# rafaelgmv/Distributed-Autonomous-Exploration-and-Mapping

Hardware: AMD Instinct MI355X
Metric: beam-cell updates/sec + frontier-extract ms on 16384² grid (higher is better)
Workload: dtype int32/u32 ray math + fp32 log-odds (fp64 endpoints)

## Files before the change

### distributed-autonomous-exploration-and-mapping_amd/csrc/dm_api.cpp

```cpp
#include <math.h>
#include <stdarg.h>
#include <stdio.h>
#include <string.h>

#include <algorithm>
#include <new>
#include <string>
#include <vector>

#include "dm_internal.h"

#include <stdlib.h>

hipError_t dm_sync_all(dm_grid* g) {
  for (hipStream_t s : {g->stream, g->fe_stream, g->pass_stream, g->big_stream}) {
    if (!s) continue;
    const hipError_t e = hipStreamSynchronize(s);
    if (e != hipSuccess) return e;
  }
  g->p_pending = false;
  for (auto& f : g->fw) f.busy_pending = false;
  return hipSuccess;
}

hipError_t dm_copy_shards(dm_grid* g) {
  const size_t bytes = sizeof(unsigned long long) * kShards * kShardWords;
  hipError_t e = hipMemcpyAsync(g->h_sh, g->iw[g->iw_cur].sh, bytes, hipMemcpyDeviceToHost, g->stream);
  if (e == hipSuccess)
    e = hipMemcpyAsync(g->h_sh + kShards * kShardWords, g->fsh, bytes, hipMemcpyDeviceToHost, g->stream);
  return e;
}

namespace {
thread_local std::string t_err;

bool dm_env_on(const char* name) {
  const char* v = getenv(name);
  return v && v[0] == '1';
}


struct HostCluster {
  long long label, size, sum_x, sum_y;
};

template <class T>
int dev_alloc(T** p, int64_t count, const char* what) {
  if (*p) { (void)hipFree(*p); *p = nullptr; }
  if (count <= 0) count = 1;
  hipError_t e = hipMalloc((void**)p, sizeof(T) * (size_t)count);
  if (e != hipSuccess) {
    *p = nullptr;
    return dm_set_error(e == hipErrorOutOfMemory ? DM_ERR_OOM : DM_ERR_HIP,
                        "hipMalloc(%s, %lld bytes): %s", what,
                        (long long)(sizeof(T) * (size_t)count), hipGetErrorString(e));
  }
  return DM_OK;
}

template <class T>
void dev_free(T*& p) {
  if (p) (void)hipFree(p);
  p = nullptr;
}

template <class T>
int dev_grow(T** p, int64_t* cap, int64_t n, const char* what) {
  if (n <= *cap) return DM_OK;
  *cap = 0;
  const int rc = dev_alloc(p, n, what);
  if (!rc) *cap = n;
  return rc;
}

int64_t ceil_div(int64_t a, int64_t b) { return (a + b - 1) / b; }

int validate_params(const dm_params* p) {
  if (!p) return dm_set_error(DM_ERR_INVALID_ARG, "params is NULL");
  if (p->width <= 0 || p->height <= 0 || p->width > (1ll << 30) || p->height > (1ll << 30))
    return dm_set_error(DM_ERR_INVALID_ARG, "width/height must be in [1, 2^30] (got %lld x %lld)",
                        (long long)p->width, (long long)p->height);
  if (!(p->resolution > 0.0) || !isfinite(p->resolution))
    return dm_set_error(DM_ERR_INVALID_ARG, "resolution must be finite and > 0");
  if (!isfinite(p->origin_x) || !isfinite(p->origin_y))
    return dm_set_error(DM_ERR_INVALID_ARG, "origin must be finite");
  if (!(p->range_min >= 0.0f) || !(p->range_max > 0.0f) || !isfinite(p->range_max))
    return dm_set_error(DM_ERR_INVALID_ARG, "need 0 <= range_min and finite range_max > 0");
  if ((double)p->range_max / p->resolution > 16384.0)
    return dm_set_error(DM_ERR_INVALID_ARG,
                        "range_max / resolution must be <= 16384 cells (rays longer than that "
                        "are outside the kernels' integer bounds)");
  if (!isfinite(p->l_occ) || !isfinite(p->l_free) || !isfinite(p->l_min) || !isfinite(p->l_max) ||
      !(p->l_min <= p->l_max))
    return dm_set_error(DM_ERR_INVALID_ARG, "log-odds constants must be finite with l_min <= l_max");
  if (isnan(p->occ_thresh) || isnan(p->free_thresh))
    return dm_set_error(DM_ERR_INVALID_ARG, "occ_thresh / free_thresh must not be NaN");
  if (p->band_row0 < 0 || p->band_row0 >= p->height || p->band_row0 % DM_TILE != 0)
    return dm_set_error(DM_ERR_INVALID_ARG, "band_row0 must be in [0, height) and a multiple of %d",
                        DM_TILE);
  int64_t R = p->band_rows > 0 ? p->band_rows : p->height - p->band_row0;
  if (R <= 0 || p->band_row0 + R > p->height)
    return dm_set_error(DM_ERR_INVALID_ARG, "band_rows out of range");
  if (ceil_div(p->width, DM_TILE) * ceil_div(R, DM_TILE) > (1ll << 30))
    return dm_set_error(DM_ERR_INVALID_ARG, "too many tiles");
  if (p->min_frontier_size < 0) return dm_set_error(DM_ERR_INVALID_ARG, "min_frontier_size < 0");
  return DM_OK;
}

int grow_integrate(dm_grid* g, int32_t S, int32_t N) {
  const int64_t nb = (int64_t)S * N;
  const int64_t chunks = dm_integrate_chunks(g, nb);
  const int64_t per_beam = 2 * (g->nmax / DM_TILE) + 8 + 4 * chunks;
  const int64_t blocks = ceil_div(nb * chunks, 256);
  if (nb > g->beams_cap || blocks > g->blk_cap) {
    const int64_t nbc = std::max<int64_t>(nb, g->beams_cap);
    const int64_t bc = std::max<int64_t>(blocks, g->blk_cap);
    int rc = 0;
    for (auto& w : g->iw) {
      if (!rc) rc = dev_alloc(&w.beams, nbc, "beams");
      if (!rc) rc = dev_alloc(&w.blk_hist, bc * 1024, "per-block tile histograms");
      if (!rc) rc = dev_alloc(&w.blk_n, bc, "per-block histogram sizes");
    }
    if (rc) { g->beams_cap = g->blk_cap = 0; return rc; }
    g->beams_cap = nbc;
    g->blk_cap = bc;
  }
  const int64_t segs = nb * per_beam;
  if (segs > g->segs_cap) {
    for (auto& w : g->iw) {
      int rc = dev_alloc(&w.pieces, segs, "ray pieces");
      if (rc) { g->segs_cap = 0; return rc; }
    }
    g->segs_cap = segs;
  }
  const int64_t side = ceil_div(2 * (int64_t)g->nmax + 1, DM_TILE) + 1;
  int64_t act = std::min<int64_t>(g->NT, std::min<int64_t>(segs, (int64_t)S * side * side));
  if (act < 1) act = 1;
  if (act > g->act_cap) {
    int rc = 0;
    for (auto& w : g->iw) {
      if (!rc) rc = dev_alloc(&w.act_raw, act * kShards, "first-touch lists");
      if (!rc) rc = dev_alloc(&w.litems, act, "light work items");
    }
    if (rc) { g->act_cap = 0; return rc; }
    g->act_cap = act;
  }
  const int64_t chunk = kIntegrateChunk;
  const int64_t heavy = std::max<int64_t>(1, std::min<int64_t>(g->act_cap, segs / (kIntegrateMedium + 1) + 1));
  const int64_t hitems = segs / chunk + segs / (chunk + 1) + 2;
  if (hitems > g->hitem_cap) {
    for (auto& w : g->iw) {
      int rc = dev_alloc(&w.hitems, hitems, "heavy work items");
      if (rc) { g->hitem_cap = 0; return rc; }
    }
    g->hitem_cap = hitems;
  }
  if (heavy > g->heavy_cap) {
    for (auto& w : g->iw) {
      int rc = dev_alloc(&w.heavy_list, heavy, "heavy tiles");
      if (!rc) rc = dev_alloc(&w.slabs, heavy * 2 * DM_TILE * DM_TILE, "heavy-tile slabs");
      if (!rc) rc = dev_alloc(&w.heavy_done, heavy, "heavy-tile item tickets");
      if (rc) { g->heavy_cap = 0; return rc; }
      DM_HIP(hipMemset(w.slabs, 0, sizeof(uint32_t) * (size_t)(heavy * 2 * DM_TILE * DM_TILE)));
      DM_HIP(hipMemset(w.heavy_done, 0, sizeof(int32_t) * (size_t)heavy));
    }
    g->heavy_cap = heavy;
  }
  if (2 * (int64_t)N > g->trig_cap) {
    int rc = dev_alloc(&g->trig, 2 * (int64_t)N, "trig table");
    if (rc) return rc;
    g->trig_cap = 2 * (int64_t)N;
    g->trig_n = -1;
  }
  return DM_OK;
}

int ensure_trig(dm_grid* g, int32_t N, float amin, float inc) {
  if (N == g->trig_n && amin == g->trig_amin && inc == g->trig_inc) return DM_OK;
  DM_HIP(dm_sync_all(g));
  std::vector<double> t(2 * (size_t)std::max(N, 1));
  for (int32_t i = 0; i < N; ++i) {
    const double phi = (double)amin + (double)i * (double)inc;
    t[2 * i] = cos(phi);
    t[2 * i + 1] = sin(phi);
  }
  if (N > 0) DM_HIP(hipMemcpy(g->trig, t.data(), sizeof(double) * 2 * N, hipMemcpyHostToDevice));
  g->trig_n = N;
  g->trig_amin = amin;
  g->trig_inc = inc;
  return DM_OK;
}

}

int dm_grow_bucket_sort(dm_grid* g, int64_t n) {
  if (n <= g->bs_cap) return DM_OK;
  int rc = dev_alloc(&g->bs_key, n, "row-sort keys");
  if (!rc) rc = dev_alloc(&g->bs_key2, n, "row-sort keys");
  if (!rc) rc = dev_alloc(&g->bs_idx, n, "row-sort indices");
  if (!rc) rc = dev_alloc(&g->bs_idx2, n, "row-sort indices");
  if (!rc && g->rs_rows < g->H) {
    rc = dev_alloc(&g->rs_cnt, g->H, "row-sort counters");
    if (!rc) rc = dev_alloc(&g->rs_off, g->H + 1, "row-sort offsets");
    if (!rc) rc = dev_alloc(&g->rs_status, g->H / 8192 + 2, "row-sort workgroup totals");
    if (!rc) {
      DM_HIP(hipMemset(g->rs_cnt, 0, sizeof(int32_t) * (size_t)g->H));
      g->rs_rows = g->H;
    }
  }
  if (rc) { g->bs_cap = 0; return rc; }
  g->bs_cap = n;
  return DM_OK;
}

namespace {

int grow_slots(dm_grid* g, int64_t need) {
  int64_t cap = std::max<int64_t>(need, 2 * g->slot_cap);
  if (cap < (1 << 16)) cap = 1 << 16;
  cap = ceil_div(cap, kShards) * kShards;
  int rc = dev_alloc(&g->slot_label, cap, "slot labels");
  for (auto& f : g->fw)
    if (!rc) rc = dev_alloc(&f.slot_parent, cap, "slot parents");
  g->slot_parent = g->fw[g->fparity].slot_parent;
  if (!rc) rc = dev_alloc(&g->slot_root, cap, "slot roots");
  if (!rc) rc = dev_alloc(&g->slot_own, 3 * cap, "slot sums");
  if (!rc) rc = dev_alloc(&g->slot_acc, 3 * cap, "slot totals");
  if (!rc) rc = dev_alloc(&g->clusters, 4 * cap, "clusters");
  for (int sl = 0; sl <= dm_grid::kRbSlots && !rc; ++sl) {
    dm_cluster* base = g->rb[sl].out_clu ? g->rb[sl].out_clu - kRbRecords : nullptr;
    rc = dev_alloc(&base, cap + kRbRecords, "sorted clusters");
    g->rb[sl].out_clu = base ? base + kRbRecords : nullptr;
  }
  ++g->rb_gen;
  g->out_clu = g->rb[g->rb_head].out_clu;
  if (!rc) rc = dev_alloc(&g->slot_k, cap, "slot cluster index");
  if (!rc) rc = dev_alloc(&g->rank_of, cap, "cluster sorted position");
  if (!rc) rc = dm_grow_bucket_sort(g, cap);
  if (rc) return rc;
  g->slot_cap = cap;
  return DM_OK;
}

int grow_host_out(dm_grid* g, int slot, int64_t need) {
  dm_grid::RbSlot& r = g->rb[slot];
  if (need <= r.h_out_cap) return DM_OK;
  int64_t cap = std::max<int64_t>(need, 2 * r.h_out_cap);
  if (r.h_out) (void)hipHostFree(r.h_out - kRbHostRecords);
  r.h_out = nullptr;
  r.h_out_cap = 0;
  dm_raw_record* base = nullptr;
  DM_HIP(hipHostMalloc((void**)&base, sizeof(dm_raw_record) * (size_t)(cap + kRbHostRecords),
                       hipHostMallocMapped | hipHostMallocCoherent));
  dm_raw_record* dbase = nullptr;
  const hipError_t e = hipHostGetDevicePointer((void**)&dbase, base, 0);
  if (e != hipSuccess) {
    (void)hipHostFree(base);
    return dm_hip_check(e, "hipHostGetDevicePointer(cluster readback)");
  }
  r.h_out = base + kRbHostRecords;
  r.h_out_dev = dbase + kRbHostRecords;
  r.h_out_cap = cap;
  return DM_OK;
}

int copy_clusters(dm_grid* g, bool sorted, int64_t n, int64_t nw, int64_t have,
                  const dm_cluster* d_sorted, const long long* d_raw, dm_cluster* out) {
  if (sorted) {
    have = std::min<int64_t>(have, nw);
    const double ox = g->p.origin_x, oy = g->p.origin_y, res = g->p.resolution;
    for (int64_t i = 0; i < have; ++i) {
      const dm_raw_record& q = g->h_out[i];
      dm_cluster& c = out[i];
      c.label = q.label;
      c.size = q.size;
      c.sum_x = q.sum_x;
      c.sum_y = q.sum_y;
      c.cx_m = dm_centroid(ox, q.sum_x, q.size, res);
      c.cy_m = dm_centroid(oy, q.sum_y, q.size, res);
    }
    if (nw > have)
      DM_HIP(hipMemcpy(out + have, d_sorted + have, sizeof(dm_cluster) * (size_t)(nw - have),
                       hipMemcpyDeviceToHost));
    return DM_OK;
  }
  std::vector<HostCluster> hc((size_t)n);
  if (n > 0) DM_HIP(hipMemcpy(hc.data(), d_raw, sizeof(HostCluster) * (size_t)n, hipMemcpyDeviceToHost));
  std::sort(hc.begin(), hc.end(), [](const HostCluster& a, const HostCluster& b) { return a.label < b.label; });
  for (int64_t i = 0; i < nw; ++i) {
    dm_cluster& c = out[i];
    c.label = hc[i].label;
    c.size = hc[i].size;
    c.sum_x = hc[i].sum_x;
    c.sum_y = hc[i].sum_y;
    c.cx_m = dm_centroid(g->p.origin_x, c.sum_x, c.size, g->p.resolution);
    c.cy_m = dm_centroid(g->p.origin_y, c.sum_y, c.size, g->p.resolution);
  }
  return DM_OK;
}

void note_goal_source(dm_grid* g, int slot, int kind, int64_t n) {
  g->goal_slot = n >= 0 ? slot : -1;
  g->goal_kind = kind;
  g->goal_n = n;
  g->goal_epoch = kind == 1 ? g->rb[slot].wepoch : g->rb[slot].mepoch;
  g->goal_gen = g->rb_gen;
}

int grow_merge(dm_grid* g, int64_t n) {
  if (n <= g->m_cap) return DM_OK;
  int rc = dev_alloc(&g->m_parent, n, "merge parents");
  if (!rc) rc = dev_alloc(&g->m_label, n, "merge labels");
  if (!rc) rc = dev_alloc(&g->m_acc, 3 * n, "merge sums");
  if (!rc) rc = dev_alloc(&g->m_clu, 4 * n, "merged clusters");
  for (int sl = 0; sl <= dm_grid::kRbSlots && !rc; ++sl)
    rc = dev_alloc(&g->rb[sl].m_out, n, "merged clusters (sorted)");
  ++g->rb_gen;
  if (!rc) rc = dm_grow_bucket_sort(g, n);
  if (rc) { g->m_cap = 0; return rc; }
  g->m_cap = n;
  return DM_OK;
}

int check_grid(const dm_grid* g) {
  if (!g) return dm_set_error(DM_ERR_INVALID_ARG, "grid handle is NULL");
  return DM_OK;
}

int not_on_sharded(const dm_grid* g, const char* what) {
  if (g && g->sh)
    return dm_set_error(DM_ERR_INVALID_ARG, "%s is not available on a sharded handle (dm_create_sharded runs "
                                            "the band exchange itself)", what);
  return DM_OK;
}

int use_device(const dm_grid* g) {
  DM_HIP(hipSetDevice(g->device));
  return DM_OK;
}

int check_integrate_args(int32_t S, int32_t N, const void* poses, const void* ranges) {
  if (S < 0 || N < 0) return dm_set_error(DM_ERR_SHAPE, "S and N must be >= 0");
  if ((int64_t)S * N > (1ll << 31) - 1) return dm_set_error(DM_ERR_SHAPE, "S*N must be < 2^31");
  if (N > 65535) return dm_set_error(DM_ERR_SHAPE, "N must be <= 65535");
  if ((int64_t)S * N > 0 && (!poses || !ranges))
    return dm_set_error(DM_ERR_INVALID_ARG, "poses/ranges is NULL");
  return DM_OK;
}

int read_counters(dm_grid* g) {
  DM_HIP(dm_join_pass_stream(g));
  DM_HIP(hipMemcpyAsync(g->h_cnt, g->cnt, sizeof(unsigned long long) * CNT_N,
                        hipMemcpyDeviceToHost, g->stream));
  DM_HIP(hipMemcpyAsync(g->h_cnt + CNT_N, g->iw[g->iw_cur].cnt, sizeof(unsigned long long) * CNT_N,
                        hipMemcpyDeviceToHost, g->stream));
  DM_HIP(hipMemcpyAsync(g->h_cnt + 2 * CNT_N, g->fe_flag + kHaltWord, sizeof(unsigned long long),
                        hipMemcpyDeviceToHost, g->stream));
  DM_HIP(dm_copy_shards(g));
  DM_HIP(hipStreamSynchronize(g->stream));
  if (g->h_cnt[2 * CNT_N])
    return dm_set_error(DM_ERR_PIPELINE, "the overlapped pipeline's front-end hand-off timed out: a map "
                        "update was skipped; dm_reset the handle");
  return DM_OK;
}

int finish_counts(dm_grid* g, uint64_t* U, uint64_t* T) {
  int rc = read_counters(g);
  if (rc) return rc;
  const unsigned long long* ic = g->h_cnt + CNT_N;
  if (ic[CNT_IOVERFLOW]) {
    (void)hipMemset(g->iw[g->iw_cur].tile_count, 0, sizeof(int32_t) * (size_t)g->NT);
    return dm_set_error(DM_ERR_CAPACITY, "integrate workspace overflow (flags %llu: 1 first-touch "
                        "list, 2 pieces, 4 work lists)",
                        (unsigned long long)ic[CNT_IOVERFLOW]);
  }
  if (U) *U = dm_shard_sum(g->h_sh, SH_U);
  if (T) *T = dm_shard_sum(g->h_sh, SH_T);
  return DM_OK;
}

}

int dm_set_error(int code, const char* fmt, ...) {
  char buf[512];
  va_list ap;
  va_start(ap, fmt);
  vsnprintf(buf, sizeof buf, fmt, ap);
  va_end(ap);
  t_err = buf;
  return code;
}

int dm_hip_check(hipError_t e, const char* what) {
  return dm_set_error(e == hipErrorOutOfMemory ? DM_ERR_OOM : DM_ERR_HIP, "%s: %s (%d)", what,
                      hipGetErrorString(e), (int)e);
}

void dm_timer_begin(dm_grid* g, const char* name, KernelTimer* t, hipStream_t s) {
  if (!g->profile) return;
  t->name = name;
  t->stream = s ? s : g->stream;
  (void)hipEventCreate(&t->start);
  (void)hipEventCreate(&t->stop);
  (void)hipEventRecord(t->start, t->stream);
}

void dm_timer_end(dm_grid* g, KernelTimer* t) {
  if (!g->profile) return;
  (void)hipEventRecord(t->stop, t->stream);
  g->pending.push_back(*t);
  if (g->pending.size() > 4096) {
    int32_t n = 0;
    (void)dm_profile_read(g, nullptr, 0, &n);
  }
}

extern "C" {

const char* dm_last_error(void) { return t_err.c_str(); }
const char* dm_version(void) { return "dm 0.1.0 (gfx950, HIP)"; }
int dm_max_passes_in_flight(void) { return dm_grid::kRbSlots; }

int dm_default_params(dm_params* p, int64_t width, int64_t height) {
  if (!p) return dm_set_error(DM_ERR_INVALID_ARG, "params is NULL");
  memset(p, 0, sizeof *p);
  p->width = width;
  p->height = height;
  p->resolution = 0.05;
  p->origin_x = -0.5 * (double)width * p->resolution;
  p->origin_y = -0.5 * (double)height * p->resolution;
  p->range_min = 0.02f;
  p->range_max = 12.0f;
  p->l_occ = 0.85f;
  p->l_free = -0.4f;
  p->l_min = -2.0f;
  p->l_max = 3.5f;
  p->occ_thresh = 0.0f;
  p->free_thresh = 0.0f;
  p->min_frontier_size = 1;
  p->band_row0 = 0;
  p->band_rows = 0;
  return DM_OK;
}

int dm_create(dm_grid** out, const dm_params* p, int device) {
  if (!out) return dm_set_error(DM_ERR_INVALID_ARG, "out is NULL");
  *out = nullptr;
  int rc = validate_params(p);
  if (rc) return rc;
  int ndev = 0;
  hipError_t e = hipGetDeviceCount(&ndev);
  if (e != hipSuccess || ndev <= 0)
    return dm_set_error(DM_ERR_HIP, "no HIP device available (%s)", hipGetErrorString(e));
  if (device < 0 || device >= ndev)
    return dm_set_error(DM_ERR_INVALID_ARG, "device %d out of range [0, %d)", device, ndev);
  DM_HIP(hipSetDevice(device));
  dm_grid* g = new (std::nothrow) dm_grid();
  if (!g) return dm_set_error(DM_ERR_OOM, "host allocation failed");
  g->p = *p;
  if (g->p.band_rows <= 0) g->p.band_rows = p->height - p->band_row0;
  g->device = device;
  g->W = p->width;
  g->H = p->height;
  g->row0 = p->band_row0;
  g->R = g->p.band_rows;
  g->TX = ceil_div(g->W, DM_TILE);
  g->TY = ceil_div(g->R, DM_TILE);
  g->NT = g->TX * g->TY;
  g->nmax = (int32_t)ceil((double)p->range_max / p->resolution) + 2;
  const int64_t cells = g->W * g->R;
  auto fail = [&](int code) {
    dm_destroy(g);
    return code;
  };
  if ((rc = dev_alloc(&g->L, cells, "log-odds"))) return fail(rc);
  if ((rc = dev_alloc(&g->state, cells, "state"))) return fail(rc);
  for (auto& w : g->iw) {
    if ((rc = dev_alloc(&w.tile_count, g->NT, "tile counts"))) return fail(rc);
    if ((rc = dev_alloc(&w.tile_cur, g->NT, "tile bin cursors"))) return fail(rc);
    if ((rc = dev_alloc(&w.cnt, CNT_N, "integrate counters"))) return fail(rc);
    if ((rc = dev_alloc(&w.sh, kShards * kShardWords, "integrate shard counters"))) return fail(rc);
    DM_HIP(hipMemset(w.cnt, 0, sizeof(unsigned long long) * CNT_N));
    DM_HIP(hipMemset(w.sh, 0, sizeof(unsigned long long) * kShards * kShardWords));
  }
  if ((rc = dev_alloc(&g->tile_free, g->NT, "tile free counts"))) return fail(rc);
  if ((rc = dev_alloc(&g->fmask, g->NT * DM_TILE * 16, "tile free / unknown bit rows"))) return fail(rc);
  if ((rc = dev_alloc(&g->fedge, g->NT * 4, "tile unknown edge words"))) return fail(rc);
  if ((rc = dev_alloc(&g->tile_seen, g->NT, "tile seen flags"))) return fail(rc);
  if (const char* sp = getenv("DM_SPARSE_PIECES")) g->sparse_pieces = std::max(0, atoi(sp));
  const char* fm = getenv("DM_FMASK");
  g->fmask_mode = fm && !strcmp(fm, "on") ? 1 : (fm && !strcmp(fm, "off") ? 2 : 0);
  const char* fk = getenv("DM_FRONTIER_KERNEL");
  g->frontier_kernel = fk && !strcmp(fk, "wave") ? 1 : (fk && !strcmp(fk, "wg") ? 2 : 0);
  if (const char* sm = getenv("DM_SORT_MIN")) g->sort_min = std::max<int64_t>(0, atoll(sm));
  g->fault_gate = dm_env_on("DM_FAULT_GATE");
  if (const char* pr = getenv("DM_PLAN_MAX_ROUNDS")) g->plan_max_rounds = std::max<int64_t>(0, atoll(pr));
  for (auto& f : g->fw) {
    e = hipEventCreateWithFlags(&f.ev_split, hipEventDisableTiming | hipEventDisableSystemFence);
    if (e != hipSuccess) return fail(dm_hip_check(e, "hipEventCreate"));
    if ((rc = dev_alloc(&f.cnt, CNT_N, "frontier counters"))) return fail(rc);
    DM_HIP(hipMemset(f.cnt, 0, sizeof(unsigned long long) * CNT_N));
    if ((rc = dev_alloc(&f.fsh, kShards * kShardWords, "frontier shard counters"))) return fail(rc);
    DM_HIP(hipMemset(f.fsh, 0, sizeof(unsigned long long) * kShards * kShardWords));
    if ((rc = dev_alloc(&f.big_tiles, g->NT, "frontier big tiles"))) return fail(rc);
    if ((rc = dev_alloc(&f.fbits, g->NT * DM_TILE, "frontier bit rows"))) return fail(rc);
    if ((rc = dev_alloc(&f.edge_slot, 2 * g->W, "edge slots"))) return fail(rc);
  }
  if ((rc = dev_alloc(&g->fl_n, 48, "frontier list lengths"))) return fail(rc);
  for (int i = 0; i < 2; ++i) {
    if ((rc = dev_alloc(&g->flist[i], g->NT, "frontier tile list"))) return fail(rc);
    if ((rc = dev_alloc(&g->flist_n[i], 16, "frontier tile list length"))) return fail(rc);
    DM_HIP(hipMemset(g->flist_n[i], 0, sizeof(unsigned long long) * 16));
  }
  g->ftiles = g->flist[0];
  g->ftiles_n = g->flist_n[0];
  DM_HIP(hipMemset(g->fl_n, 0, sizeof(unsigned long long) * 48));
  if ((rc = dev_alloc(&g->bits_flag, 16, "bit-row hand-off word"))) return fail(rc);
  DM_HIP(hipMemset(g->bits_flag, 0, sizeof(unsigned long long) * 16));
  if ((rc = dev_alloc(&g->fe_flag, 16, "front-end completion words"))) return fail(rc);
  DM_HIP(hipMemset(g->fe_flag, 0, sizeof(unsigned long long) * 16));
  if ((rc = dev_alloc(&g->border, g->NT * 256, "frontier borders"))) return fail(rc);
  if ((rc = dev_alloc(&g->rel, 8 * g->NT, "tile-edge hand-off words"))) return fail(rc);
  DM_HIP(hipMemset(g->rel, 0, sizeof(unsigned long long) * 8 * (size_t)g->NT));
  if ((rc = dev_alloc(&g->edge_label, 2 * g->W, "edge labels"))) return fail(rc);
  if ((rc = dev_alloc(&g->halo, 2 * g->W, "halo rows"))) return fail(rc);
  if ((rc = grow_slots(g, std::max<int64_t>(1 << 16, kSlotsPerTile * g->NT)))) return fail(rc);
  dm_select_fw(g, g->fparity);
  for (int sl = 0; sl <= dm_grid::kRbSlots; ++sl)
    if ((rc = grow_host_out(g, sl, 1 << 14))) return fail(rc);
  dm_select_slot(g, 0);
  e = hipHostMalloc((void**)&g->h_cnt, sizeof(unsigned long long) * (2 * CNT_N + 1), hipHostMallocDefault);
  if (e != hipSuccess) return fail(dm_hip_check(e, "hipHostMalloc(counters)"));
  e = hipHostMalloc((void**)&g->h_sh, sizeof(unsigned long long) * 2 * kShards * kShardWords,
                    hipHostMallocDefault);
  if (e != hipSuccess) return fail(dm_hip_check(e, "hipHostMalloc(shard counters)"));
  if ((rc = dev_alloc(&g->m_cnt, 4, "merge counters"))) return fail(rc);
  e = hipHostMalloc((void**)&g->h_mcnt, sizeof(unsigned long long) * 4, hipHostMallocDefault);
  if (e != hipSuccess) return fail(dm_hip_check(e, "hipHostMalloc(merge counters)"));
  e = hipHostMalloc((void**)&g->h_hint, sizeof(unsigned long long) * 16, hipHostMallocMapped | hipHostMallocCoherent);
  if (e != hipSuccess) return fail(dm_hip_check(e, "hipHostMalloc(work hint)"));
  memset(g->h_hint, 0, sizeof(unsigned long long) * 16);
  e = hipHostGetDevicePointer((void**)&g->d_hint, g->h_hint, 0);
  if (e != hipSuccess) return fail(dm_hip_check(e, "hipHostGetDevicePointer(work hint)"));
  e = hipDeviceGetAttribute(&g->n_cu, hipDeviceAttributeMultiprocessorCount, device);
  if (e != hipSuccess) return fail(dm_hip_check(e, "hipDeviceGetAttribute(multiprocessor count)"));
  int prio_lo = 0, prio_hi = 0;
  (void)hipDeviceGetStreamPriorityRange(&prio_lo, &prio_hi);
  e = hipStreamCreateWithPriority(&g->stream, hipStreamNonBlocking, prio_hi);
  if (e != hipSuccess) return fail(dm_hip_check(e, "hipStreamCreate"));
  g->own_stream = true;
  e = hipStreamCreateWithPriority(&g->fe_stream, hipStreamNonBlocking, prio_lo);
  if (e != hipSuccess) return fail(dm_hip_check(e, "hipStreamCreate(front-end)"));
  e = hipStreamCreateWithPriority(&g->pass_stream, hipStreamNonBlocking, prio_hi);
  if (e != hipSuccess) return fail(dm_hip_check(e, "hipStreamCreate(pass)"));
  e = hipStreamCreateWithPriority(&g->big_stream, hipStreamNonBlocking, prio_hi);
  if (e != hipSuccess) return fail(dm_hip_check(e, "hipStreamCreate(big)"));
  for (hipEvent_t* ev : {&g->ev_fe, &g->ev_bits[0], &g->ev_bits[1], &g->iw[0].ev_free, &g->iw[1].ev_free,
                         &g->ev_bigfork, &g->ev_big, &g->flist_ev[0], &g->flist_ev[1]}) {
    e = hipEventCreateWithFlags(ev, hipEventDisableTiming | hipEventDisableSystemFence);
    if (e != hipSuccess) return fail(dm_hip_check(e, "hipEventCreate"));
  }
  for (auto& r : g->rb) {
    e = hipEventCreateWithFlags(&r.ev, hipEventDisableTiming);
    if (e != hipSuccess) return fail(dm_hip_check(e, "hipEventCreate"));
  }
  for (hipEvent_t& ev : g->ev_pose) {
    e = hipEventCreateWithFlags(&ev, hipEventDisableTiming);
    if (e != hipSuccess) return fail(dm_hip_check(e, "hipEventCreate"));
  }

  if ((rc = dm_reset(g))) return fail(rc);
  *out = g;
  return DM_OK;
}

int dm_destroy(dm_grid* g) {
  if (g && g->sh) return dm_sh_destroy(g);
  if (!g) return DM_OK;
  (void)hipSetDevice(g->device);
  (void)dm_sync_all(g);
  for (auto& t : g->pending) { (void)hipEventDestroy(t.start); (void)hipEventDestroy(t.stop); }
  for (hipEvent_t ev : {g->ev_fe, g->ev_bits[0], g->ev_bits[1], g->iw[0].ev_free, g->iw[1].ev_free,
                        g->ev_bigfork, g->ev_big, g->flist_ev[0], g->flist_ev[1]})
    if (ev) (void)hipEventDestroy(ev);
  for (auto& r : g->rb) {
    if (r.ev) (void)hipEventDestroy(r.ev);
    if (r.out_clu) (void)hipFree(r.out_clu - kRbRecords);
    if (r.h_out) (void)hipHostFree(r.h_out - kRbHostRecords);
    dev_free(r.m_out);
  }
  if (g->fe_stream) (void)hipStreamDestroy(g->fe_stream);
  if (g->pass_stream) (void)hipStreamDestroy(g->pass_stream);
  if (g->big_stream) (void)hipStreamDestroy(g->big_stream);
  for (auto& f : g->fw) {
    if (f.ev_split) (void)hipEventDestroy(f.ev_split);
    dev_free(f.cnt); dev_free(f.fsh); dev_free(f.big_tiles); dev_free(f.fbits);
    dev_free(f.edge_slot); dev_free(f.slot_parent);
  }
  dev_free(g->fl_n); dev_free(g->bits_flag);
  for (int i = 0; i < 2; ++i) { dev_free(g->flist[i]); dev_free(g->flist_n[i]); }
  for (int b = 0; b < 2; ++b) { dev_free(g->goal_k[b]); dev_free(g->goal_i[b]); }
  dev_free(g->goal_io); dev_free(g->goal_idx);
  dev_free(g->plan_cost); dev_free(g->plan_trav); dev_free(g->plan_travs); dev_free(g->plan_list[0]);
  dev_free(g->plan_list[1]); dev_free(g->plan_stamp); dev_free(g->plan_len); dev_free(g->plan_stat);
  dev_free(g->plan_src); dev_free(g->plan_qxy); dev_free(g->plan_qcost); dev_free(g->plan_qcell);
  dev_free(g->plan_path);
  if (g->h_plan) (void)hipHostFree(g->h_plan);
  dev_free(g->match_V); dev_free(g->match_kern); dev_free(g->match_tiles); dev_free(g->match_pose4);
  dev_free(g->match_trig); dev_free(g->match_ranges); dev_free(g->match_q); dev_free(g->match_vol);
  dev_free(g->match_out);
  for (auto& w : g->iw) {
    dev_free(w.pieces); dev_free(w.hitems); dev_free(w.litems); dev_free(w.heavy_list); dev_free(w.slabs);
    dev_free(w.heavy_done); dev_free(w.tile_count); dev_free(w.tile_cur); dev_free(w.cnt); dev_free(w.sh);
    dev_free(w.ranges);
    dev_free(w.beams); dev_free(w.blk_hist); dev_free(w.blk_n); dev_free(w.act_raw);
  }
  dev_free(g->L); dev_free(g->state); dev_free(g->fmask); dev_free(g->fedge); dev_free(g->tile_seen);
  dev_free(g->tile_free);
  dev_free(g->trig);
  dev_free(g->bs_key); dev_free(g->bs_key2); dev_free(g->bs_idx); dev_free(g->bs_idx2);
  dev_free(g->rs_cnt); dev_free(g->rs_off); dev_free(g->rs_status);
  dev_free(g->border); dev_free(g->rel); dev_free(g->slot_label); dev_free(g->slot_root);
  dev_free(g->slot_own); dev_free(g->slot_acc); dev_free(g->clusters); dev_free(g->cell_slot);
  dev_free(g->edge_label); dev_free(g->mask); dev_free(g->labels);
  dev_free(g->halo); dev_free(g->fe_flag);
  dev_free(g->slot_k); dev_free(g->rank_of); dev_free(g->m_parent); dev_free(g->m_label);
  dev_free(g->m_acc); dev_free(g->m_clu); dev_free(g->m_cnt);
  if (g->h_mcnt) (void)hipHostFree(g->h_mcnt);
  if (g->h_hint) (void)hipHostFree(g->h_hint);
  if (g->h_cnt) (void)hipHostFree(g->h_cnt);
  if (g->h_sh) (void)hipHostFree(g->h_sh);
  for (int i = 0; i < dm_grid::kPoseRing; ++i) {
    if (g->h_pose4[i]) (void)hipHostFree(g->h_pose4[i]);
    if (g->ev_pose[i]) (void)hipEventDestroy(g->ev_pose[i]);
  }
  if (g->stream && g->own_stream) (void)hipStreamDestroy(g->stream);
  delete g;
  return DM_OK;
}

int dm_reset(dm_grid* g) {
  if (g && g->sh) return dm_sh_reset(g);
  int rc = check_grid(g);
  if (rc || (rc = use_device(g))) return rc;
  const int64_t cells = g->W * g->R;
  DM_HIP(hipMemsetAsync(g->L, 0, sizeof(float) * (size_t)cells, g->stream));
  DM_HIP(hipMemsetAsync(g->state, 0xFF, (size_t)cells, g->stream));
  DM_HIP(dm_sync_all(g));
  for (auto& w : g->iw) DM_HIP(hipMemsetAsync(w.tile_count, 0, sizeof(int32_t) * (size_t)g->NT, g->stream));
  DM_HIP(hipMemsetAsync(g->tile_free, 0, sizeof(int32_t) * (size_t)g->NT, g->stream));
  if ((rc = dm_launch_recount(g))) return rc;
  for (auto& f : g->fw) DM_HIP(hipMemsetAsync(f.cnt, 0, sizeof(unsigned long long) * CNT_N, g->stream));
  DM_HIP(hipMemsetAsync(g->fe_flag + kHaltWord, 0, sizeof(unsigned long long), g->stream));
  DM_HIP(hipStreamSynchronize(g->stream));
  ++g->reset_seq;
  return DM_OK;
}

int dm_get_params(const dm_grid* g, dm_params* out) {
  int rc = check_grid(g);
  if (rc) return rc;
  if (!out) return dm_set_error(DM_ERR_INVALID_ARG, "out is NULL");
  *out = g->p;
  return DM_OK;
}

}

namespace {

int enqueue_host_integrate(dm_grid* g, int32_t S, const double* poses, int32_t N, const float* ranges,
                           float angle_min, float angle_increment) {
  int rc = 0;
  if ((rc = check_integrate_args(S, N, poses, ranges))) return rc;
  if ((rc = grow_integrate(g, S, N))) return rc;
  if ((rc = ensure_trig(g, N, angle_min, angle_increment))) return rc;
  const int64_t nb = (int64_t)S * N;
  hipStream_t fs = g->overlap ? g->fe_stream : g->stream;
  dm_grid::IntWs& w = g->iw[dm_next_set(g)];
  if (g->overlap) {
    DM_HIP(dm_mark_ws_free(g));
    DM_HIP(hipStreamWaitEvent(fs, w.free_wait ? w.free_wait : w.ev_free, 0));
  }
  if (nb > w.ranges_cap || (int64_t)S * 4 > g->h_pose_cap) {
    DM_HIP(dm_sync_all(g));
  }
  if (nb > w.ranges_cap) {
    if ((rc = dev_alloc(&w.ranges, nb, "ranges"))) return rc;
    w.ranges_cap = nb;
  }
  if ((int64_t)S * 4 > g->h_pose_cap) {
    for (int i = 0; i < dm_grid::kPoseRing; ++i) {
      if (g->h_pose4[i]) (void)hipHostFree(g->h_pose4[i]);
      g->h_pose4[i] = nullptr;
    }
    g->h_pose_cap = 0;
    for (int i = 0; i < dm_grid::kPoseRing; ++i) {
      DM_HIP(hipHostMalloc((void**)&g->h_pose4[i], sizeof(double) * 4 * (size_t)std::max(S, 1),
                           hipHostMallocMapped | hipHostMallocCoherent));
      DM_HIP(hipHostGetDevicePointer((void**)&g->h_pose4_dev[i], g->h_pose4[i], 0));
    }
    g->h_pose_cap = (int64_t)std::max(S, 1) * 4;
  }
  const int slot = g->pose_head;
  g->pose_head = (g->pose_head + 1) % dm_grid::kPoseRing;
  DM_HIP(hipEventSynchronize(g->ev_pose[slot]));
  double* hp = g->h_pose4[slot];
  for (int32_t s = 0; s < S; ++s) {
    const double x = poses[3 * s], y = poses[3 * s + 1], yaw = poses[3 * s + 2];
    hp[4 * s + 0] = x;
    hp[4 * s + 1] = y;
    hp[4 * s + 2] = cos(yaw);
    hp[4 * s + 3] = sin(yaw);
  }
  if (nb > 0)
    DM_HIP(hipMemcpyAsync(w.ranges, ranges, sizeof(float) * (size_t)nb, hipMemcpyHostToDevice, fs));
  if ((rc = dm_launch_integrate(g, S, g->h_pose4_dev[slot], N, w.ranges, g->trig))) return rc;
  DM_HIP(hipEventRecord(g->ev_pose[slot], fs));
  g->last_S = S;
  g->last_N = N;
  g->frontier_valid = false;
  ++g->integrate_seq;
  return DM_OK;
}

}

extern "C" {

int dm_integrate(dm_grid* g, int32_t S, const double* poses, int32_t N, const float* ranges,
                 float angle_min, float angle_increment, uint64_t* out_updates,
                 uint64_t* out_touched) {
  if (g && g->sh) return dm_sh_integrate(g, S, poses, N, ranges, angle_min, angle_increment, out_updates, out_touched);
  int rc = check_grid(g);
  if (rc || (rc = use_device(g))) return rc;
  if ((rc = enqueue_host_integrate(g, S, poses, N, ranges, angle_min, angle_increment))) return rc;
  return finish_counts(g, out_updates, out_touched);
}

int dm_integrate_async(dm_grid* g, int32_t S, const double* poses, int32_t N, const float* ranges,
                       float angle_min, float angle_increment) {
  if (g && g->sh) return dm_sh_integrate_async(g, S, poses, N, ranges, angle_min, angle_increment);
  int rc = check_grid(g);
  if (rc || (rc = use_device(g))) return rc;
  return enqueue_host_integrate(g, S, poses, N, ranges, angle_min, angle_increment);
}

int dm_integrate_device(dm_grid* g, int32_t S, const double* d_pose4, int32_t N,
                        const float* d_ranges, float angle_min, float angle_increment) {
  if (g && g->sh) return dm_sh_integrate_device(g, S, d_pose4, N, d_ranges, angle_min, angle_increment);
  int rc = check_grid(g);
  if (rc || (rc = use_device(g))) return rc;
  if ((rc = check_integrate_args(S, N, d_pose4, d_ranges))) return rc;
  if ((rc = grow_integrate(g, S, N))) return rc;
  if ((rc = ensure_trig(g, N, angle_min, angle_increment))) return rc;
  if ((rc = dm_launch_integrate(g, S, d_pose4, N, d_ranges, g->trig))) return rc;
  g->last_S = S;
  g->last_N = N;
  g->frontier_valid = false;
  ++g->integrate_seq;
  return DM_OK;
}

int dm_last_counts(dm_grid* g, uint64_t* updates, uint64_t* touched) {
  if (g && g->sh) return dm_sh_last_counts(g, updates, touched);
  int rc = check_grid(g);
  if (rc || (rc = use_device(g))) return rc;
  return finish_counts(g, updates, touched);
}

int dm_last_stats(dm_grid* g, uint64_t* out, int32_t cap, int32_t* n_out) {
  if (g && g->sh) return dm_sh_last_stats(g, out, cap, n_out);
  int rc = check_grid(g);
  if (rc || (rc = use_device(g))) return rc;
  if (cap > 0 && !out) return dm_set_error(DM_ERR_INVALID_ARG, "out is NULL");
  if ((rc = read_counters(g))) return rc;
  const unsigned long long* fs = g->h_sh + kShards * kShardWords;
  const unsigned long long* ic = g->h_cnt + CNT_N;
  const uint64_t items = ic[CNT_ITEMS] + ic[CNT_LITEMS] + ic[CNT_SITEMS];
  const uint64_t pieces = ic[CNT_SEGS];
  const uint64_t v[kNStats] = {dm_shard_sum(g->h_sh, SH_U),  dm_shard_sum(g->h_sh, SH_T),
                               dm_shard_sum(g->h_sh, SH_TH), pieces,
                               ic[CNT_ACTIVE],               items,
                               ic[CNT_HEAVY],                g->h_cnt[CNT_FL0],
                               dm_shard_sum(fs, SH_SLOT),    g->h_cnt[CNT_CLUSTERS],
                               ic[CNT_SITEMS]};
  for (int32_t i = 0; i < cap && i < kNStats; ++i) out[i] = v[i];
  if (n_out) *n_out = kNStats;
  return DM_OK;
}

int dm_get_state(dm_grid* g, int8_t* out) {
  if (g && g->sh) return (out ? dm_sh_get_state(g, out) : dm_set_error(DM_ERR_INVALID_ARG, "out is NULL"));
  int rc = check_grid(g);
  if (rc || (rc = use_device(g))) return rc;
  if (!out) return dm_set_error(DM_ERR_INVALID_ARG, "out is NULL");
  DM_HIP(hipMemcpyAsync(out, g->state, (size_t)(g->W * g->R), hipMemcpyDeviceToHost, g->stream));
  DM_HIP(hipStreamSynchronize(g->stream));
  return DM_OK;
}

int dm_get_logodds(dm_grid* g, float* out) {
  if (g && g->sh) return (out ? dm_sh_get_logodds(g, out) : dm_set_error(DM_ERR_INVALID_ARG, "out is NULL"));
  int rc = check_grid(g);
  if (rc || (rc = use_device(g))) return rc;
  if (!out) return dm_set_error(DM_ERR_INVALID_ARG, "out is NULL");
  DM_HIP(hipMemcpyAsync(out, g->L, sizeof(float) * (size_t)(g->W * g->R), hipMemcpyDeviceToHost,
                        g->stream));
  DM_HIP(hipStreamSynchronize(g->stream));
  return DM_OK;
}

int dm_set_logodds(dm_grid* g, const float* in) {
  if (g && g->sh) return (in ? dm_sh_set_logodds(g, in) : dm_set_error(DM_ERR_INVALID_ARG, "in is NULL"));
  int rc = check_grid(g);
  if (rc || (rc = use_device(g))) return rc;
  if (!in) return dm_set_error(DM_ERR_INVALID_ARG, "in is NULL");
  DM_HIP(hipStreamSynchronize(g->stream));
  DM_HIP(hipMemcpy(g->L, in, sizeof(float) * (size_t)(g->W * g->R), hipMemcpyHostToDevice));
  if ((rc = dm_launch_state_from_logodds(g))) return rc;
  DM_HIP(hipStreamSynchronize(g->stream));
  g->frontier_valid = false;
  ++g->integrate_seq;
  return DM_OK;
}

int dm_set_state(dm_grid* g, const int8_t* in) {
  if (g && g->sh) return (in ? dm_sh_set_state(g, in) : dm_set_error(DM_ERR_INVALID_ARG, "in is NULL"));
  int rc = check_grid(g);
  if (rc || (rc = use_device(g))) return rc;
  if (!in) return dm_set_error(DM_ERR_INVALID_ARG, "in is NULL");
  const int64_t cells = g->W * g->R;
  int8_t* d = nullptr;
  if ((rc = dev_alloc(&d, cells, "state staging"))) return rc;
  DM_HIP(hipStreamSynchronize(g->stream));
  hipError_t e = hipMemcpy(d, in, (size_t)cells, hipMemcpyHostToDevice);
  if (e == hipSuccess) {
    rc = dm_launch_set_state(g, d);
    if (!rc) e = hipStreamSynchronize(g->stream);
  }
  (void)hipFree(d);
  if (e != hipSuccess) return dm_hip_check(e, "dm_set_state");
  g->frontier_valid = false;
  ++g->integrate_seq;
  return rc;
}

int dm_frontiers(dm_grid* g, uint8_t* mask, int64_t* labels, dm_cluster* out, int64_t cap,
                 int64_t* n_out) {
  if (g && g->sh) return dm_sh_frontiers(g, mask, labels, out, cap, n_out);
  int rc = check_grid(g);
  if (rc || (rc = use_device(g))) return rc;
  if (cap < 0 || (cap > 0 && !out)) return dm_set_error(DM_ERR_INVALID_ARG, "bad cluster buffer");
  const int64_t cells = g->W * g->R;
  if (mask && !g->mask && (rc = dev_alloc(&g->mask, cells, "dense mask"))) return rc;
  if (labels && !g->cell_slot) {
    if ((rc = dev_alloc(&g->cell_slot, cells, "dense cell slots"))) return rc;
    if ((rc = dev_alloc(&g->labels, cells, "dense labels"))) return rc;
  }
  const int slot = dm_grid::kRbSync;
  dm_select_slot(g, slot);
  int64_t n = 0, copied = 0;
  for (int attempt = 0; attempt < 8; ++attempt) {
    rc = dm_launch_frontiers(g, mask != nullptr, labels != nullptr, &n, &copied);
    if (rc != DM_ERR_CAPACITY) break;
    if ((rc = grow_slots(g, n + n / 2 + 1024))) return rc;
    rc = DM_ERR_CAPACITY;
  }
  if (rc) return rc == DM_ERR_CAPACITY ? dm_set_error(rc, "frontier slot arrays kept overflowing") : rc;
  g->frontier_valid = true;
  const int64_t nw = std::min<int64_t>(n, cap);
  note_goal_source(g, slot, 1, g->h_cnt[CNT_SORTED] != 0 ? n : -1);
  if ((rc = copy_clusters(g, g->h_cnt[CNT_SORTED] != 0, n, nw, copied, g->out_clu, g->clusters, out)))
    return rc;
  if ((rc = grow_host_out(g, slot, n + n / 4 + 64))) return rc;
  if (mask) DM_HIP(hipMemcpy(mask, g->mask, (size_t)cells, hipMemcpyDeviceToHost));
  if (labels) DM_HIP(hipMemcpy(labels, g->labels, sizeof(int64_t) * (size_t)cells, hipMemcpyDeviceToHost));
  if (n_out) *n_out = n;
  if (n > cap) return dm_set_error(DM_ERR_CAPACITY, "%lld clusters, capacity %lld", (long long)n,
                                   (long long)cap);
  return DM_OK;
}

int dm_export_bytes(const dm_grid* g, int64_t rec_cap, int64_t* bytes) {
  if (int rc0 = not_on_sharded(g, "dm_export_bytes")) return rc0;
  int rc = check_grid(g);
  if (rc) return rc;
  if (!bytes || rec_cap < 0) return dm_set_error(DM_ERR_INVALID_ARG, "bytes is NULL or rec_cap < 0");
  *bytes = dm_export_nbytes(g->W, rec_cap);
  return DM_OK;
}

int dm_frontiers_export_device(dm_grid* g, void* d_export, int64_t rec_cap) {
  if (int rc0 = not_on_sharded(g, "dm_frontiers_export_device")) return rc0;
  int rc = check_grid(g);
  if (rc || (rc = use_device(g))) return rc;
  if (!d_export || rec_cap < 0) return dm_set_error(DM_ERR_INVALID_ARG, "d_export is NULL or rec_cap < 0");
  if (g->p.min_frontier_size > 1)
    return dm_set_error(DM_ERR_INVALID_ARG,
                        "export needs a band handle with min_frontier_size <= 1 (the size filter "
                        "applies to merged clusters)");
  dm_select_slot(g, g->rb_count < dm_grid::kRbSlots ? (g->rb_head + g->rb_count) % dm_grid::kRbSlots
                                                    : dm_grid::kRbSync);
  hipStream_t es = g->stream;
  if ((rc = dm_enqueue_frontiers(g, false, false, g->overlap, &es))) return rc;
  if ((rc = dm_launch_export(g, es, d_export, rec_cap))) return rc;
  if (es != g->stream) {
    dm_grid::FrWs& f = g->fw[g->fparity];
    DM_HIP(hipEventRecord(f.ev_split, es));
    f.busy = f.ev_split;
    f.busy_pending = true;
    f.busy_pass = g->fr_pass;
    g->p_tail = f.ev_split;
    g->p_pending = true;
    g->p_tail_pass = g->fr_pass;
  } else {
    DM_HIP(dm_mark_ws_free(g));
  }
  g->frontier_valid = true;
  return DM_OK;
}

int dm_exchange_stream(dm_grid* g, void** stream) {
  if (int rc0 = not_on_sharded(g, "dm_exchange_stream")) return rc0;
  int rc = check_grid(g);
  if (rc) return rc;
  if (!stream) return dm_set_error(DM_ERR_INVALID_ARG, "stream is NULL");
  *stream = (void*)dm_exchange_stream_of(g);
  return DM_OK;
}

namespace {

int claim_slot(dm_grid* g, int* slot) {
  if (g->rb_count == dm_grid::kRbSlots)
    return dm_set_error(DM_ERR_INVALID_ARG, "%d passes in flight: end the oldest first", dm_grid::kRbSlots);
  *slot = (g->rb_head + g->rb_count) % dm_grid::kRbSlots;
  dm_select_slot(g, *slot);
  return DM_OK;
}

int wait_oldest(dm_grid* g, int kind, const char* what) {
  if (!g->rb_count || g->rb[g->rb_head].kind != kind)
    return dm_set_error(DM_ERR_INVALID_ARG, "the oldest pass in flight is not a %s pass", what);
  DM_HIP(dm_event_wait(g->rb[g->rb_head].ev));
  if (kind == 1) {
    const uint64_t pass = g->rb[g->rb_head].pass;
    for (auto& f : g->fw)
      if (f.busy_pending && f.busy_pass <= pass) f.busy_pending = false;
    if (g->p_pending && g->p_tail_pass <= pass) g->p_pending = false;
  }
  dm_select_slot(g, g->rb_head);
// ... 941 lines not shown
```

### distributed-autonomous-exploration-and-mapping_amd/csrc/dm_integrate.hip

```cpp
#include "dm_internal.h"
#include "dm_phase.h"

#include <algorithm>

DM_PH_DECL(integrate)
DM_TL_DECL(accum)

namespace {

constexpr int kLdsPitch = DM_TS + 1;

struct Geom {
  RayGeom r;
  int32_t act_cap;
  int64_t seg_cap;
  int64_t hitem_cap, heavy_cap;
  int64_t nb;
  int32_t chunks, chunk_len;
  int32_t sparse_pieces;
  int32_t pad;
};

struct BeamChunk {
  int64_t b;
  int32_t k_lo, k_hi;
};

__device__ inline BeamChunk beam_chunk(const Geom& g, int64_t v) {
  BeamChunk c;
  if (g.chunks == 1) {
    c.b = v; c.k_lo = 0; c.k_hi = 0x7FFFFFFF;
    return c;
  }
  const int32_t q = (int32_t)(v / g.nb);
  c.b = v - (int64_t)q * g.nb;
  c.k_lo = q * g.chunk_len;
  c.k_hi = q + 1 == g.chunks ? 0x7FFFFFFF : c.k_lo + g.chunk_len - 1;
  return c;
}

__device__ inline int lane_id() { return __lane_id(); }

constexpr int kHash = 1024;
constexpr int kProbe = 32;

__device__ inline uint32_t tile_hash(int32_t t) { return ((uint32_t)t * 2654435761u) >> 22; }

__device__ inline int hash_insert(int32_t* hkey, int32_t tile) {
  uint32_t h = tile_hash(tile);
  for (int p = 0; p < kProbe; ++p, h = (h + 1) & (kHash - 1)) {
    const int32_t k = atomicCAS(&hkey[h], -1, tile);
    if (k == -1 || k == tile) return (int)h;
  }
  return -1;
}

__device__ inline int hash_find(const int32_t* hkey, int32_t tile) {
  uint32_t h = tile_hash(tile);
  for (int p = 0; p < kProbe; ++p, h = (h + 1) & (kHash - 1)) {
    const int32_t k = hkey[h];
    if (k == tile) return (int)h;
    if (k == -1) return -1;
  }
  return -1;
}

struct LaneRun {
  bool head;
  int head_lane;
  int len;
  int rank;
};

__device__ inline LaneRun lane_run(int32_t tile) {
  const int lane = lane_id();
  const unsigned long long act = __ballot(1);
  const int32_t prev = __shfl_up(tile, 1);
  const bool prev_act = lane > 0 && ((act >> (lane - 1)) & 1ull);
  const bool head = !(prev_act && prev == tile);
  const unsigned long long heads = __ballot(head);
  const unsigned long long le = lane == 63 ? ~0ull : ((2ull << lane) - 1ull);
  LaneRun r;
  r.head = head;
  r.head_lane = 63 - __clzll(heads & le);
  const unsigned long long after = heads & ~le;
  const unsigned long long before_end = after ? ((1ull << (__ffsll(after) - 1)) - 1ull) : ~0ull;
  const unsigned long long from_head = ~((1ull << r.head_lane) - 1ull);
  r.len = __popcll(act & from_head & before_end);
  r.rank = __popcll(act & from_head & ((1ull << lane) - 1ull));
  return r;
}

__device__ inline void first_touch(const Geom& g, int32_t tile, int32_t old, int32_t* act_raw,
                                   unsigned long long* ish, unsigned long long* cnt) {
  if (old != 0) return;
  const int sh = blockIdx.x % kShards;
  const unsigned long long l = atomicAdd(&ish[sh * kShardWords + SH_ACT], 1ull);
  if (l < (unsigned long long)g.act_cap) act_raw[(int64_t)sh * g.act_cap + (int64_t)l] = tile;
  else atomicOr(&cnt[CNT_IOVERFLOW], 1ull);
}

__device__ inline PackedPiece make_piece(const Geom& g, const Beam& bm, int32_t tile, int32_t k0, int32_t k1) {
  const int32_t tx0 = (tile % g.r.TX) * DM_TS;
  const int32_t ty0 = (tile / g.r.TX) * DM_TS;
  return dm_pack_piece(dm_tile_piece(bm, k0, k1, g.r.row0, tx0, ty0, kLdsPitch));
}

__global__ __launch_bounds__(256) void k_beam_prep(RayArgs a, Geom g, const double* __restrict__ pose4,
                                                   const float* __restrict__ ranges,
                                                   const double* __restrict__ trig,
                                                   Beam* __restrict__ beams, int32_t* tile_count,
                                                   int32_t* act_raw, unsigned long long* ish,
                                                   int2* __restrict__ blk_hist, int32_t* __restrict__ blk_n,
                                                   unsigned long long* cnt) {
  __shared__ int32_t hkey[kHash];
  __shared__ int32_t hcnt[kHash];
  __shared__ int32_t s_nh;
  const int tid = threadIdx.x;
  for (int e = tid; e < kHash; e += 256) { hkey[e] = -1; hcnt[e] = 0; }
  if (tid == 0) s_nh = 0;
  __syncthreads();
  const int64_t v = (int64_t)blockIdx.x * blockDim.x + tid;
  if (v < g.nb * g.chunks) {
    const BeamChunk bc = beam_chunk(g, v);
    const int32_t s = (int32_t)(bc.b / a.N), i = (int32_t)(bc.b % a.N);
    const Beam bm = dm_make_beam(a, pose4, ranges, trig, s, i);
    if (bc.k_lo == 0) beams[bc.b] = bm;
    if ((bm.flags & 1) && bc.k_lo <= bm.n) {
      dm_for_each_piece(bm, g.r, [&](int32_t tile, int32_t, int32_t) {
        const LaneRun run = lane_run(tile);
        if (run.head) {
          const int h = hash_insert(hkey, tile);
          if (h >= 0) {
            atomicAdd(&hcnt[h], run.len);
          } else {
            const int32_t old = atomicAdd(&tile_count[tile], run.len);
            first_touch(g, tile, old, act_raw, ish, cnt);
          }
        }
      }, bc.k_lo, bc.k_hi);
    }
  }
  __syncthreads();
  int2* my_hist = blk_hist + (int64_t)blockIdx.x * kHash;
  for (int e = tid; e < kHash; e += 256) {
    const int32_t tile = hkey[e];
    if (tile < 0) continue;
    const int32_t old = atomicAdd(&tile_count[tile], hcnt[e]);
    first_touch(g, tile, old, act_raw, ish, cnt);
    my_hist[atomicAdd(&s_nh, 1)] = make_int2(tile, hcnt[e] | (e << 16));
  }
  __syncthreads();
  if (tid == 0) blk_n[blockIdx.x] = s_nh;
}

constexpr int kChunk = kIntegrateChunk;
constexpr int kMedium = kIntegrateMedium;
static_assert(kMedium < 65536, "packed 16-bit LDS counts of medium tiles");
constexpr int kTileWords = DM_TS * kLdsPitch;
constexpr int kQuarter = 256;
static_assert(kChunk < 65536, "packed 16-bit LDS counts");
static_assert(kChunk == kQuarter, "one piece per thread");


constexpr int kPlanThreads = 256;

template <int K>
__device__ inline void wave_alloc_n(unsigned long long* const (&counter)[K], const unsigned long long (&v)[K],
                                    unsigned long long (&out)[K]) {
  const int lane = __lane_id();
  unsigned long long incl[K], total[K], base[K];
#pragma unroll
  for (int k = 0; k < K; ++k) {
    incl[k] = v[k];
    for (int d = 1; d < 64; d <<= 1) {
      const unsigned long long t = __shfl_up(incl[k], d);
      if (lane >= d) incl[k] += t;
    }
    total[k] = __shfl(incl[k], 63);
    base[k] = 0ull;
  }
  const int kk = 63 - lane;
  unsigned long long* addr = counter[0];
  unsigned long long mine = 0ull;
#pragma unroll
  for (int k = 0; k < K; ++k)
    if (kk == k) { addr = counter[k]; mine = total[k]; }
  unsigned long long got = 0ull;
  if (kk < K) got = atomicAdd(addr, mine);
#pragma unroll
  for (int k = 0; k < K; ++k) {
    base[k] = __shfl(got, 63 - k);
    out[k] = base[k] + incl[k] - v[k];
  }
}

__global__ __launch_bounds__(kPlanThreads) void k_plan(Geom g, const int32_t* __restrict__ act_raw,
                                                       const unsigned long long* __restrict__ ish,
                                                       int32_t* __restrict__ tile_cur,
                                                       const int32_t* __restrict__ tile_count,
                                                       int4* __restrict__ hitems, int4* __restrict__ litems,
                                                       int32_t* __restrict__ heavy_list,
                                                       unsigned long long* cnt) {
  __shared__ int32_t soff[kShards + 1];
  const int tid = threadIdx.x, lane = __lane_id();
  if (tid < 64) {
    const int32_t c = tid < kShards ? (int32_t)min((unsigned long long)g.act_cap, ish[tid * kShardWords + SH_ACT]) : 0;
    int32_t incl = c;
    for (int d = 1; d < 64; d <<= 1) {
      const int32_t t = __shfl_up(incl, d);
      if (lane >= d) incl += t;
    }
    if (tid < kShards) soff[tid] = incl - c;
    if (tid == kShards - 1) soff[kShards] = incl;
  }
  __syncthreads();
  const int64_t n = min((int64_t)soff[kShards], (int64_t)g.act_cap);
  if (blockIdx.x == 0 && tid == 0) cnt[CNT_ACTIVE] = (unsigned long long)n;
  const int64_t stride = (int64_t)gridDim.x * blockDim.x;
  for (int64_t j0 = (int64_t)blockIdx.x * blockDim.x + (tid & ~63); j0 < n; j0 += stride) {
    const int64_t j = j0 + lane;
    int32_t t = -1, c = 0;
    if (j < n) {
      int a = 0, b = kShards - 1;
      while (a < b) {
        const int mid = (a + b + 1) >> 1;
        if (soff[mid] <= j) a = mid; else b = mid - 1;
      }
      t = act_raw[(int64_t)a * g.act_cap + (j - soff[a])];
      c = tile_count[t];
    }
    const bool heavy = c > kMedium;
    const bool medium = c > kChunk && !heavy;
    const bool sparse = t >= 0 && c <= g.sparse_pieces;
    const bool light = t >= 0 && c <= kChunk && !sparse;
    const int32_t nh_items = heavy ? (c + kChunk - 1) / kChunk : (medium ? 1 : 0);
    unsigned long long* const ctr[5] = {&cnt[CNT_SEGS], &cnt[CNT_ITEMS], &cnt[CNT_LITEMS], &cnt[CNT_SITEMS],
                                        &cnt[CNT_HEAVY]};
    const unsigned long long want[5] = {(unsigned long long)c, (unsigned long long)nh_items, light ? 1ull : 0ull,
                                        sparse ? 1ull : 0ull, heavy ? 1ull : 0ull};
    unsigned long long got[5];
    wave_alloc_n<5>(ctr, want, got);
    const unsigned long long p0 = got[0], hi = got[1], li = got[2], si = got[3], ho = got[4];
    if (t < 0) continue;
    tile_cur[t] = (int32_t)p0;
    const bool fits = (int64_t)(p0 + c) <= g.seg_cap && (int64_t)(hi + nh_items) <= g.hitem_cap &&
                      (int64_t)li < (int64_t)g.act_cap && (int64_t)si < (int64_t)g.act_cap &&
                      (int64_t)ho < g.heavy_cap;
    if (!fits) {
      atomicOr(&cnt[CNT_IOVERFLOW], 4ull);
      continue;
    }
    if (sparse) {
      litems[(int64_t)g.act_cap - 1 - (int64_t)si] = make_int4(t, (int32_t)p0, c, -1);
    } else if (light) {
      litems[li] = make_int4(t, (int32_t)p0, c, -1);
    } else if (medium) {
      hitems[hi] = make_int4(t, (int32_t)p0, c, -1);
    } else {
      const int32_t wide = c >= 65536 ? 1 : 0;
      heavy_list[ho] = t | (wide << 31);
      for (int32_t q = 0; q < nh_items; ++q)
        hitems[hi + q] = make_int4(t, (int32_t)p0 + q * kChunk, min(kChunk, c - q * kChunk),
                                   (int32_t)(2 * ho + wide));
    }
  }
}

__device__ inline void put_piece(const Geom& g, PackedPiece* pieces, int64_t idx, const Beam& bm,
                                 int32_t tile, int32_t k0, int32_t k1, unsigned long long* cnt) {
  if (idx >= 0 && idx < g.seg_cap) {
    pieces[idx] = make_piece(g, bm, tile, k0, k1);
  } else {
    atomicOr(&cnt[CNT_IOVERFLOW], 2ull);
  }
}

__global__ __launch_bounds__(256) void k_scatter(RayArgs a, Geom g, const Beam* __restrict__ beams,
                                                 int32_t* tile_cur, const int2* __restrict__ blk_hist,
                                                 const int32_t* __restrict__ blk_n,
                                                 PackedPiece* __restrict__ pieces, unsigned long long* cnt) {
  __shared__ int32_t hkey[kHash];
  __shared__ int32_t hcnt[kHash];
  __shared__ int32_t hbase[kHash];
  const int tid = threadIdx.x;
  for (int e = tid; e < kHash; e += 256) { hkey[e] = -1; hcnt[e] = 0; }
  const int64_t v = (int64_t)blockIdx.x * blockDim.x + tid;
  const bool in = v < g.nb * g.chunks;
  const BeamChunk bc = beam_chunk(g, in ? v : 0);
  Beam bm;
  bm.flags = 0;
  if (in) bm = beams[bc.b];
  const int32_t nh = blk_n[blockIdx.x];
  __syncthreads();
  const int2* my_hist = blk_hist + (int64_t)blockIdx.x * kHash;
  for (int e = tid; e < nh; e += 256) {
    const int2 te = my_hist[e];
    const int h = hash_insert(hkey, te.x);
    if (h >= 0) hbase[h] = atomicAdd(&tile_cur[te.x], te.y & 0xFFFF);
  }
  __syncthreads();
  const bool valid = in && (bm.flags & 1) && bc.k_lo <= bm.n;
  if (valid) {
    dm_for_each_piece(bm, g.r, [&](int32_t tile, int32_t k0, int32_t k1) {
      const LaneRun run = lane_run(tile);
      int32_t pos = -1;
      if (run.head) {
        const int h = hash_find(hkey, tile);
        pos = h >= 0 ? hbase[h] + atomicAdd(&hcnt[h], run.len) : atomicAdd(&tile_cur[tile], run.len);
      }
      pos = __shfl(pos, run.head_lane);
      put_piece(g, pieces, (int64_t)pos + run.rank, bm, tile, k0, k1, cnt);
    }, bc.k_lo, bc.k_hi);
  }
}

struct ApplyArgs {
  float l_occ, l_free, l_min, l_max, occ_t, free_t;
};

__device__ inline int8_t state_of(const ApplyArgs& p, float L) {
  int32_t r = -1;
  r = L <= p.free_t ? 0 : r;
  r = L >= p.occ_t ? 100 : r;
  r = L == 0.0f ? -1 : r;
  return (int8_t)r;
}

__device__ inline float apply_one(const ApplyArgs& p, float L, uint32_t h, uint32_t m) {
  const float t = (float)h * p.l_occ;
  const float u = (float)m * p.l_free;
  L = L + t;
  L = L + u;
  return __builtin_amdgcn_fmed3f(L, p.l_min, p.l_max);
}

__device__ inline uint32_t nz_mask(uint32_t x) {
  uint32_t r;
  asm("v_min_u32_e32 %0, 1, %1\n\tv_sub_u32_e32 %0, 0, %0" : "=&v"(r) : "v"(x));
  return r;
}
__device__ inline uint32_t bfi(uint32_t m, uint32_t a, uint32_t b) {
  uint32_t r;
  asm("v_bfi_b32 %0, %1, %2, %3" : "=v"(r) : "v"(m), "v"(a), "v"(b));
  return r;
}
__device__ inline uint32_t state_bits(const ApplyArgs& p, float L) {
  const int32_t sge = (int32_t)__float_as_uint(L - p.occ_t) >> 31;
  const int32_t sle = (int32_t)__float_as_uint(p.free_t - L) >> 31;
  const int32_t mz = (int32_t)((__float_as_uint(L) & 0x7FFFFFFFu) - 1u) >> 31;
  uint32_t s = bfi((uint32_t)sle, 0xFFFFFFFFu, 0u);
  s = bfi((uint32_t)sge, s, 100u);
  return s | (uint32_t)mz;
}

__device__ inline uint8_t state_nibbles(uint32_t w) {
  auto zb = [](uint32_t v) {
    uint32_t t = (v & 0x7F7F7F7Fu) + 0x7F7F7F7Fu;
    t = ~(t | v | 0x7F7F7F7Fu);
    return (((t >> 7) * 0x00204081u) >> 21) & 0xFu;
  };
  return (uint8_t)(zb(w) | (zb(~w) << 4));
}

template <class G>
__device__ inline uint8_t state_nibbles_at(const G& g, const int8_t* __restrict__ state, int32_t x0, int32_t y) {
  uint32_t fn = 0u, un = 0u;
  for (int e = 0; e < 4; ++e) {
    if (x0 + e >= g.r.W) break;
    const int8_t b = state[(int64_t)y * g.r.W + x0 + e];
    fn |= (b == 0 ? 1u : 0u) << e;
    un |= (b == -1 ? 1u : 0u) << e;
  }
  return (uint8_t)(fn | (un << 4));
}

__device__ inline uint32_t every4th(uint64_t x) {
  x &= 0x1111111111111111ull;
  x = (x | (x >> 3)) & 0x0303030303030303ull;
  x = (x | (x >> 6)) & 0x000F000F000F000Full;
  x = (x | (x >> 12)) & 0x000000FF000000FFull;
  return (uint32_t)((x | (x >> 24)) & 0xFFFFull);
}

struct EdgeAcc {
  uint64_t w[4] = {0ull, 0ull, 0ull, 0ull};
};
__device__ inline void edge_acc(EdgeAcc& e, uint32_t out, int q, int lane) {
  const int c = lane & 3;
  const uint64_t b0 = __ballot(c == 0 && ((out >> 4) & 1u));
  const uint64_t b3 = __ballot(c == 3 && ((out >> 31) & 1u));
  e.w[0] |= (uint64_t)every4th(b0) << (16 * q);
  e.w[1] |= (uint64_t)every4th(b3 >> 3) << (16 * q);
  if (q == 0 || q == 3) {
    const uint32_t u16 = ((out >> 4) & 0xFu) | ((out >> 8) & 0xF0u) | ((out >> 12) & 0xF00u) | ((out >> 16) & 0xF000u);
    const int base = q == 0 ? 0 : 60;
    uint64_t r = 0ull;
#pragma unroll
    for (int k = 0; k < 4; ++k) r |= (uint64_t)__shfl(u16, base + k) << (16 * k);
    e.w[q == 0 ? 2 : 3] = r;
  }
}

__device__ inline void edge_store(const EdgeAcc& e, uint64_t* __restrict__ fedge, int64_t tile, uint64_t rows,
                                  int lane) {
  if (lane >= 4) return;
  const uint64_t v = lane == 0 ? e.w[0] : lane == 1 ? e.w[1] : lane == 2 ? e.w[2] : e.w[3];
  const uint64_t m = lane < 2 ? rows : ((rows >> (lane == 2 ? 0 : 63)) & 1ull) ? ~0ull : 0ull;
  uint64_t* p = fedge + tile * 4 + lane;
  if (m == ~0ull) *p = v;
  else if (m) *p = (*p & ~m) | (v & m);
}

__device__ inline int32_t zero_bytes(uint32_t x) {
  uint32_t t = (x & 0x7F7F7F7Fu) + 0x7F7F7F7Fu;
  t = ~(t | x | 0x7F7F7F7Fu);
  return __popc(t);
}

template <int ROWS>
struct CellRows {
  float4 l[ROWS];
  char4 s[ROWS];
  bool vec;

  __device__ void prefetch(const Geom& g, int32_t tx0, int32_t ty0, int ly0, int dly, int cx,
                           const float* __restrict__ L, const int8_t* __restrict__ state, int vec_ok) {
    vec = vec_ok && tx0 + cx + 4 <= g.r.W;
#pragma unroll
    for (int rr = 0; rr < ROWS; ++rr) {
      const int32_t y = ty0 + ly0 + rr * dly;
      const int64_t base = (vec && y < g.r.R) ? (int64_t)y * g.r.W + tx0 + cx : 0;
      l[rr] = *reinterpret_cast<const float4*>(L + base);
      s[rr] = *reinterpret_cast<const char4*>(state + base);
    }
  }

  template <class Touched>
  __device__ void load_touched(const Geom& g, int32_t tx0, int32_t ty0, int ly0, int dly, int cx,
                               const float* __restrict__ L, const int8_t* __restrict__ state, int vec_ok,
                               Touched&& touched) {
    vec = vec_ok && tx0 + cx + 4 <= g.r.W;
#pragma unroll
    for (int rr = 0; rr < ROWS; ++rr) {
      const int32_t y = ty0 + ly0 + rr * dly;
      l[rr] = make_float4(0.0f, 0.0f, 0.0f, 0.0f);
      s[rr] = make_char4(0, 0, 0, 0);
      if (vec && y < g.r.R && touched(ly0 + rr * dly)) {
        const int64_t base = (int64_t)y * g.r.W + tx0 + cx;
        l[rr] = *reinterpret_cast<const float4*>(L + base);
        s[rr] = *reinterpret_cast<const char4*>(state + base);
      }
    }
  }

  template <class Counts>
  __device__ void apply(const Geom& g, const ApplyArgs& p, int32_t tx0, int32_t ty0, int ly0, int dly,
                        int cx, float* __restrict__ L, int8_t* __restrict__ state, Counts&& counts,
                        int32_t* sh_T, int32_t* sh_free, uint32_t* sh_U) {
    int32_t dT = 0, dFree = 0;
    uint32_t dU = 0;
#pragma unroll
    for (int rr = 0; rr < ROWS; ++rr) {
      const int ly = ly0 + rr * dly;
      const int32_t y = ty0 + ly;
      if (y >= g.r.R) continue;
      uint32_t h4[4], m4[4];
      counts(ly, h4, m4);
      if (((h4[0] | m4[0]) | (h4[1] | m4[1]) | (h4[2] | m4[2]) | (h4[3] | m4[3])) == 0u) continue;
      const int64_t base = (int64_t)y * g.r.W + tx0 + cx;
      if (sh_U) {
#pragma unroll
        for (int e = 0; e < 4; ++e) dU += tx0 + cx + e < g.r.W ? h4[e] + m4[e] : 0u;
      }
      if (vec) {
        const float lv[4] = {l[rr].x, l[rr].y, l[rr].z, l[rr].w};
        const uint32_t sw = *reinterpret_cast<const uint32_t*>(&s[rr]);
        uint32_t nlb[4], nsw = 0u, msk = 0u;
#pragma unroll
        for (int e = 0; e < 4; ++e) {
          const uint32_t mh = nz_mask(h4[e] | m4[e]);
          const float nl = apply_one(p, lv[e], h4[e], m4[e]);
          nlb[e] = bfi(mh, __float_as_uint(nl), __float_as_uint(lv[e]));
          nsw |= (state_bits(p, nl) & 0xFFu) << (8 * e);
          msk |= (mh & 0xFFu) << (8 * e);
          dT += (int32_t)(mh & 1u);
        }
        const uint32_t ns = bfi(msk, nsw, sw);
        dFree += zero_bytes(ns) - zero_bytes(sw);
        *reinterpret_cast<float4*>(L + base) =
            make_float4(__uint_as_float(nlb[0]), __uint_as_float(nlb[1]), __uint_as_float(nlb[2]),
                        __uint_as_float(nlb[3]));
        *reinterpret_cast<uint32_t*>(state + base) = ns;
      } else {
        for (int e = 0; e < 4; ++e) {
          if ((h4[e] | m4[e]) == 0u || tx0 + cx + e >= g.r.W) continue;
          const int64_t i = base + e;
          const int8_t old = state[i];
          const float nl = apply_one(p, L[i], h4[e], m4[e]);
          const int8_t ns = state_of(p, nl);
          L[i] = nl;
          state[i] = ns;
          dT += 1;
          dFree += (ns == 0) - (old == 0);
        }
      }
    }
    if (dT) atomicAdd(sh_T, dT);
    if (dFree) atomicAdd(sh_free, dFree);
    if (dU) atomicAdd(sh_U, dU);
  }
};

__device__ inline int32_t walk_tp(uint32_t* tl, const TilePiece& tp, int32_t len, int lane) {
  int32_t wl = len;
  for (int o = 32; o > 0; o >>= 1) wl = max(wl, __shfl_xor(wl, o));
  const int32_t s0 = len > 0 ? lane % len : 0;
  PieceCursor cur;
  cur.init(tp);
  if (s0 > 0) {
    const int32_t num = tp.rem0 + s0 * tp.two_adb;
    const int32_t dq = dm_udiv_small(num, tp.two_n, __builtin_amdgcn_rcpf((float)tp.two_n));
    cur.addr = tp.addr0 + s0 * tp.da + dq * tp.db;
    cur.rem = num - dq * tp.two_n;
  }
  int32_t k = s0;
  for (int32_t st = 0; st < wl; ++st) {
    if (st < len) {
      atomicAdd(&tl[cur.addr], 1u);
      cur.step(tp);
      if (++k == len) cur.init(tp);
    }
  }
  if (len > 0 && tp.addr_end >= 0) atomicAdd(&tl[tp.addr_end], 0xFFFFu);
  return len;
}

__device__ inline int32_t walk_piece(uint32_t* tl, const PackedPiece& mine, bool valid, int lane) {
  const TilePiece tp = dm_unpack_piece(mine.x, mine.y, mine.z, mine.w);
  return walk_tp(tl, tp, valid ? tp.len : 0, lane);
}

__device__ inline int32_t walk_tp_split(uint32_t* tl, const TilePiece& tp, int32_t len, int32_t f, int32_t part,
                                        float rf, int lane) {
  const SplitPart sp = dm_split_part(len, f, part, rf);
  int32_t wl = sp.n;
  for (int o = 32; o > 0; o >>= 1) wl = max(wl, __shfl_xor(wl, o));
  const int32_t spare = kTileWords + lane;
  PieceCursor cur;
  if (f == 1) cur.init(tp);
  else cur.init_at(tp, sp.j0, __builtin_amdgcn_rcpf((float)tp.two_n));
  for (int32_t st = 0; st < wl; ++st) {
    atomicAdd(&tl[st < sp.n ? cur.addr : spare], 1u);
    cur.step(tp);
  }
  if (sp.n > 0 && sp.j0 + sp.n == len && tp.addr_end >= 0) atomicAdd(&tl[tp.addr_end], 0xFFFFu);
  return sp.n;
}

constexpr int kSparseMax = 15;
#ifndef DM_SPARSE_LIST
#define DM_SPARSE_LIST 256
#endif
constexpr int kSparseList = DM_SPARSE_LIST;

__device__ inline int32_t to_pitch64(int32_t a) {
  return a >= 0 ? a - a / kLdsPitch : -((-a) - (-a) / kLdsPitch);
}

__device__ inline int32_t walk_piece_bytes(uint32_t* tq, const PackedPiece& mine, bool valid, int32_t f,
                                           int32_t part, float rf) {
  TilePiece tp = dm_unpack_piece(mine.x, mine.y, mine.z, mine.w);
  const int32_t len = valid ? tp.len : 0;
  const SplitPart sp = dm_split_part(len, f, part, rf);
  int32_t wl = sp.n;
  for (int o = 32; o > 0; o >>= 1) wl = max(wl, __shfl_xor(wl, o));
  tp.addr0 = to_pitch64(tp.addr0);
  tp.da = to_pitch64(tp.da);
  tp.db = to_pitch64(tp.db);
  PieceCursor cur;
  if (f == 1) cur.init(tp);
  else cur.init_at(tp, sp.j0, __builtin_amdgcn_rcpf((float)tp.two_n));
  for (int32_t st = 0; st < wl; ++st) {
    if (st < sp.n) atomicAdd(&tq[cur.addr >> 2], 1u << (8 * (cur.addr & 3)));
    cur.step(tp);
  }
  if (sp.n > 0 && sp.j0 + sp.n == len && tp.addr_end >= 0) {
    const int32_t e = to_pitch64(tp.addr_end);
    atomicAdd(&tq[e >> 2], 0x0Fu << (8 * (e & 3)));
  }
  return sp.n;
}

__device__ inline PackedPiece no_piece() {
  PackedPiece q;
  q.x = 0u; q.y = 0u; q.z = 0u; q.w = 1u;
  return q;
}

__device__ inline int32_t free_update(int32_t old, int32_t dfree, int32_t tile, int32_t* tlist,
                                      unsigned long long* tlist_n) {
  int32_t v = old + dfree;
  if (dfree > 0 && !(old & kTileListed)) {
    v |= kTileListed;
    tlist[atomicAdd(tlist_n, 1ull)] = tile;
  }
  return v;
}

__device__ inline void finish_tile(const Geom& g, int32_t tile, int32_t T, int32_t dfree, uint32_t U,
                                   bool heavy, int32_t* tile_count, int32_t* tile_free, int32_t old_free,
                                   int32_t* tlist, unsigned long long* tlist_n, unsigned long long* ish) {
  unsigned long long* sh = ish + (blockIdx.x % kShards) * kShardWords;
  if (T) {
    atomicAdd(&sh[SH_T], (unsigned long long)T);
    if (heavy) atomicAdd(&sh[SH_TH], (unsigned long long)T);
  }
  if (U) atomicAdd(&sh[SH_U], (unsigned long long)U);
  if (dfree) tile_free[tile] = free_update(old_free, dfree, tile, tlist, tlist_n);
  tile_count[tile] = 0;
}

__device__ inline void heavy_quarter(const Geom& g, const ApplyArgs& p, int64_t h, int q, int32_t tile,
                                     bool wide, uint32_t* __restrict__ slabs, float* __restrict__ L,
                                     int8_t* __restrict__ state, int32_t* s_T, int32_t* s_free,
                                     uint32_t* s_U) {
  constexpr int kQ = DM_TS * DM_TS / 4;
  const int tid = threadIdx.x;
  const int32_t x = (tile % g.r.TX) * DM_TS + (tid & 63);
  const int32_t yq = (tile / g.r.TX) * DM_TS + q * (DM_TS / 4) + (tid >> 6);
  uint32_t* sh = slabs + h * (2 * DM_TS * DM_TS) + q * kQ + tid;
  uint32_t hc[4], mc[4];
  float lv[4];
  int8_t sv[4];
#pragma unroll
  for (int k = 0; k < 4; ++k) {
    const int32_t y = yq + 4 * k;
    lv[k] = 0.0f;
    sv[k] = 0;
    if (y < g.r.R && x < g.r.W) {
      lv[k] = L[(int64_t)y * g.r.W + x];
      sv[k] = state[(int64_t)y * g.r.W + x];
    }
  }
#pragma unroll
  for (int k = 0; k < 4; ++k) {
    hc[k] = atomicExch(sh + k * kQuarter, 0u);
    mc[k] = wide ? atomicExch(sh + DM_TS * DM_TS + k * kQuarter, 0u) : 0u;
  }
  int32_t dT = 0, dFree = 0;
  uint32_t dU = 0;
#pragma unroll
  for (int k = 0; k < 4; ++k) {
    uint32_t hk = hc[k], mk;
    if (wide) {
      mk = mc[k];
    } else {
      mk = hk & 0xFFFFu;
      hk >>= 16;
    }
    const int32_t y = yq + 4 * k;
    if ((hk | mk) == 0u || y >= g.r.R || x >= g.r.W) continue;
    const int64_t i = (int64_t)y * g.r.W + x;
    const float nl = apply_one(p, lv[k], hk, mk);
    const int8_t ns = state_of(p, nl);
    L[i] = nl;
    state[i] = ns;
    dU += hk + mk;
    dT += 1;
    dFree += (ns == 0) - (sv[k] == 0);
  }
  if (dT) atomicAdd(s_T, dT);
  if (dFree) atomicAdd(s_free, dFree);
  if (dU) atomicAdd(s_U, dU);
}

#ifndef DM_ACCUM_OCC
#define DM_ACCUM_OCC 7
#endif
constexpr int kAccumPerCu = DM_ACCUM_OCC;
__global__ __launch_bounds__(kQuarter, kAccumPerCu) void k_tile_accum(
    Geom g, ApplyArgs p, const int4* __restrict__ list_a, int cnt_a, const int4* __restrict__ list_b,
    int cnt_b, int cnt_c, const PackedPiece* __restrict__ pieces, int32_t* tile_count, int32_t* tile_free,
    uint32_t* __restrict__ slabs, float* __restrict__ L, int8_t* __restrict__ state,
    const unsigned long long* __restrict__ cnt, unsigned long long* ish, int vec_ok,
    const int32_t* __restrict__ heavy_list, int32_t* heavy_done, int32_t* tlist, unsigned long long* tlist_n,
    unsigned long long* hint, const unsigned long long* __restrict__ halt, uint8_t* __restrict__ tile_seen) {
  __shared__ uint32_t tl[kTileWords + 64];
  __shared__ int32_t s_T, s_free, s_last;
  __shared__ uint32_t s_U;
  const int tid = threadIdx.x, lane = lane_id();
  DM_TL_BEGIN();
  const unsigned long long hv = *halt;
  const unsigned long long ca = cnt[cnt_a];
  const unsigned long long cb = cnt[cnt_b];
  const unsigned long long cc = cnt[cnt_c];
  const int64_t HI = min((int64_t)ca, g.hitem_cap);
  const int64_t LI = min((int64_t)cb, (int64_t)g.act_cap);
  const int64_t n_items = HI + LI;
  const int64_t SI = min((int64_t)cc, (int64_t)g.act_cap);
  const int64_t G = gridDim.x;
  const int64_t sp_rank = ((int64_t)blockIdx.x - n_items % G + G) % G;
  if (blockIdx.x == 0 && tid == 0) {
    volatile unsigned long long* h = hint;
    h[0] = (unsigned long long)(n_items + (SI + 3) / 4);
    h[1] = (unsigned long long)(n_items + SI);
  }
  const unsigned long long idle =
      ((int64_t)blockIdx.x >= n_items && sp_rank * (kQuarter / 64) >= SI) ? 1ull : 0ull;
  if ((hv | idle) != 0ull) {
    DM_TL_END(accum, 0);
    return;
  }
  auto item_of = [&](int64_t it) {
    int4 d = it < n_items ? (it < HI ? list_a[it] : list_b[it - HI]) : make_int4(0, 0, 0, -1);
    d.z = (int64_t)d.y + d.z <= g.seg_cap ? d.z : 0;
    return d;
  };
  const int cx = (tid & 15) * 4;
  __shared__ unsigned long long s_accT, s_accU;
  int4 info = item_of(blockIdx.x);
  int4 next = item_of(blockIdx.x + G);
  PackedPiece mine;
  CellRows<4> cells;
  int32_t tfree;
  auto split_of = [&](const int4& d) -> int32_t {
    const int32_t c = __builtin_amdgcn_readfirstlane(d.z);
    const int32_t heavy = __builtin_amdgcn_readfirstlane(d.w);
    return heavy < 0 ? dm_split_factor(c, kQuarter) : 1;
  };
  auto piece_of = [&](int32_t f) -> int32_t {
    return f == 1 ? tid : dm_udiv_small(tid, f, __builtin_amdgcn_rcpf((float)f));
  };
  auto load_pieces = [&](const int4& d) -> PackedPiece {
    const int32_t c0 = __builtin_amdgcn_readfirstlane(d.y);
    const int32_t c = __builtin_amdgcn_readfirstlane(d.z);
    return pieces[c0 + min(piece_of(split_of(d)), max(c - 1, 0))];
  };
  mine = load_pieces(info);
  PackedPiece mine_n = mine;
  for (int e = tid; e < kTileWords; e += kQuarter) tl[e] = 0u;
  if (tid == 0) { s_T = 0; s_free = 0; s_U = 0u; s_accT = 0ull; s_accU = 0ull; }
  __syncthreads();
  DM_PH_INIT();
  [[maybe_unused]] unsigned long long tl_word = 0;
  for (int64_t it = blockIdx.x; it < n_items; it += G) {
    tl_word += 1;
    const int32_t tile = __builtin_amdgcn_readfirstlane(info.x);
    const int32_t c0 = __builtin_amdgcn_readfirstlane(info.y);
    const int32_t c = __builtin_amdgcn_readfirstlane(info.z);
    const int32_t heavy = __builtin_amdgcn_readfirstlane(info.w);
    const int32_t tx0 = (tile % g.r.TX) * DM_TS, ty0 = (tile / g.r.TX) * DM_TS;
    DM_PH(dm_phase_acc_integrate, 0);
    if (heavy >= 0) {
      walk_piece(tl, mine, tid < c, lane);
      mine_n = load_pieces(next);
      __syncthreads();
      DM_PH(dm_phase_acc_integrate, 1);
      DM_PH_COUNT(dm_phase_acc_integrate, 17, 1);
      DM_PH_COUNT(dm_phase_acc_integrate, 19, c);
      uint32_t* sh = slabs + (int64_t)(heavy >> 1) * (2 * DM_TS * DM_TS);
      if (heavy & 1) {
        for (int e = tid; e < DM_TS * DM_TS; e += kQuarter) {
          const uint32_t v = tl[(e >> 6) * kLdsPitch + (e & 63)];
          const uint32_t h = v >> 16, m = v & 0xFFFFu;
          if (h) atomicAdd(&sh[e], h);
          if (m) atomicAdd(&sh[DM_TS * DM_TS + e], m);
        }
      } else {
        for (int e = tid; e < DM_TS * DM_TS; e += kQuarter) {
          const uint32_t v = tl[(e >> 6) * kLdsPitch + (e & 63)];
          if (v) atomicAdd(&sh[e], v);
        }
      }
      DM_PH(dm_phase_acc_integrate, 2);
      asm volatile("s_waitcnt vmcnt(0)" ::: "memory");
      __syncthreads();
      if (tid == 0) {
        const int32_t n_it = (tile_count[tile] + kChunk - 1) / kChunk;
        s_last = atomicAdd(&heavy_done[heavy >> 1], 1) == n_it - 1;
      }
      __syncthreads();
      if (s_last) {
#ifdef DM_PHASE_TIMING
        const long long tf0 = wall_clock64();
#endif
        const int64_t h = heavy >> 1;
        const bool wide = heavy_list[h] < 0;
        const int32_t old_free = tid == 0 ? tile_free[tile] : 0;
        for (int q = 0; q < 4; ++q)
          heavy_quarter(g, p, h, q, tile, wide, slabs, L, state, &s_T, &s_free, &s_U);
        __syncthreads();
        if (tid == 0) {
          finish_tile(g, tile, s_T, s_free, s_U, true, tile_count, tile_free, old_free, tlist, tlist_n, ish);
          heavy_done[h] = 0;
          tile_seen[tile] = 1;
        }
#ifdef DM_PHASE_TIMING
        tl_word += (unsigned long long)(wall_clock64() - tf0) << 32;
#endif
      }
    } else {
      tfree = tile_free[tile];
      cells.prefetch(g, tx0, ty0, tid >> 4, 16, cx, L, state, vec_ok);
      int32_t u;
      if (c <= kChunk) {
        const int32_t f = split_of(info);
        const int32_t pi = piece_of(f);
        const TilePiece tp = dm_unpack_piece(mine.x, mine.y, mine.z, mine.w);
        u = walk_tp_split(tl, tp, pi < c ? tp.len : 0, f, tid - pi * f, __builtin_amdgcn_rcpf((float)f), lane);
      } else {
        u = walk_piece(tl, mine, tid < c, lane);
        for (int32_t r0 = kChunk; r0 < c; r0 += kChunk) {
          const PackedPiece more = r0 + tid < c ? pieces[c0 + r0 + tid] : no_piece();
          u += walk_piece(tl, more, r0 + tid < c, lane);
        }
      }
      const bool inside = tx0 + DM_TS <= g.r.W && ty0 + DM_TS <= g.r.R;
      if (inside) {
        for (int o = 32; o > 0; o >>= 1) u += __shfl_xor(u, o);
        if (lane == 0) atomicAdd(&s_U, (uint32_t)u);
      }
      mine_n = load_pieces(next);
      __syncthreads();
      DM_PH(dm_phase_acc_integrate, 3);
      DM_PH_COUNT(dm_phase_acc_integrate, 16, 1);
      DM_PH_COUNT(dm_phase_acc_integrate, 18, c);
      cells.apply(g, p, tx0, ty0, tid >> 4, 16, cx, L, state,
                  [&](int ly, uint32_t* h4, uint32_t* m4) {
                    for (int e = 0; e < 4; ++e) {
                      const uint32_t v = tl[ly * kLdsPitch + cx + e];
                      h4[e] = v >> 16;
                      m4[e] = v & 0xFFFFu;
                    }
                  },
                  &s_T, &s_free, inside ? nullptr : &s_U);
      DM_PH(dm_phase_acc_integrate, 4);
    }
    __syncthreads();
    if (tid == 0 && heavy < 0) {
      s_accT += (unsigned long long)s_T;
      s_accU += (unsigned long long)s_U;
      if (s_free) tile_free[tile] = free_update(tfree, s_free, tile, tlist, tlist_n);
      tile_count[tile] = 0;
      tile_seen[tile] = 1;
    }
    info = next;
    next = item_of(it + 2 * G);
    mine = mine_n;
    for (int e = tid; e < kTileWords; e += kQuarter) tl[e] = 0u;
    if (tid == 0) { s_T = 0; s_free = 0; s_U = 0u; }
    __syncthreads();
  }
  __shared__ int32_t s_wT[kQuarter / 64], s_wfree[kQuarter / 64];
  __shared__ uint32_t s_wU[kQuarter / 64];
  __shared__ uint16_t s_list[kQuarter / 64][kSparseList];
  const int wv = tid >> 6;
  uint32_t* tq = tl + wv * (DM_TS * DM_TS / 4);
  const int hcx = (lane & 15) * 4;
  if (lane == 0) { s_wT[wv] = 0; s_wfree[wv] = 0; s_wU[wv] = 0u; }
  const int nw = kQuarter / 64;
  for (int64_t it = sp_rank * nw + wv; it < SI; it += (int64_t)G * nw) {
    int4 d = list_b[(int64_t)g.act_cap - 1 - it];
    d.z = (int64_t)d.y + d.z <= g.seg_cap ? d.z : 0;
    const int32_t tile = d.x, c0 = d.y, c = d.z;
    if (lane == 0 && wv == 0) tl_word += 1ull << 16;
    const int32_t tx0 = (tile % g.r.TX) * DM_TS, ty0 = (tile / g.r.TX) * DM_TS;
    const int32_t fs = dm_split_factor(c, 64);
    const float rfs = __builtin_amdgcn_rcpf((float)fs);
    const int32_t spi = fs == 1 ? lane : dm_udiv_small(lane, fs, rfs);
    const PackedPiece sp = spi < c ? pieces[c0 + spi] : no_piece();
    const int32_t sfree = tile_free[tile];
    int32_t u = walk_piece_bytes(tq, sp, spi < c, fs, lane - spi * fs, rfs);
    const bool inside = tx0 + DM_TS <= g.r.W && ty0 + DM_TS <= g.r.R;
    uint32_t wU = 0u;
    if (inside) {
      for (int o = 32; o > 0; o >>= 1) u += __shfl_xor(u, o);
      wU = (uint32_t)u;
    }
    __builtin_amdgcn_fence(__ATOMIC_ACQ_REL, "wavefront");
    __builtin_amdgcn_wave_barrier();
    DM_PH(dm_phase_acc_integrate, 6);
    auto counts = [&](int wi, uint32_t* h4, uint32_t* m4) {
      const uint32_t w = tq[wi];
      for (int e = 0; e < 4; ++e) {
        const uint32_t v = (w >> (8 * e)) & 0xFFu;
        h4[e] = v >> 4;
        m4[e] = v & 0xFu;
      }
    };
    uint16_t* lst = s_list[wv];
    int nt = 0;
    {
      const unsigned long long lt = (1ull << lane) - 1ull;
#pragma unroll
      for (int k = 0; k < 16; ++k) {
        const int wi = k * 64 + lane;
        const bool nz = tq[wi] != 0u;
        const unsigned long long m = __ballot(nz);
        const int at = nt + __popcll(m & lt);
        if (nz && at < kSparseList) lst[at] = (uint16_t)wi;
        nt += __popcll(m);
      }
    }
    __builtin_amdgcn_fence(__ATOMIC_ACQ_REL, "wavefront");
    __builtin_amdgcn_wave_barrier();
    if (nt <= kSparseList) {
      for (int e0 = 0; e0 < nt; e0 += 128) {
        const int ea = e0 + lane, eb = e0 + 64 + lane;
        const int wa = ea < nt ? lst[ea] : 0, wb = eb < nt ? lst[eb] : 0;
        CellRows<1> ca, cb;
        ca.load_touched(g, tx0, ty0, wa >> 4, 0, (wa & 15) * 4, L, state, vec_ok, [&](int) { return ea < nt; });
        cb.load_touched(g, tx0, ty0, wb >> 4, 0, (wb & 15) * 4, L, state, vec_ok, [&](int) { return eb < nt; });
        if (ea < nt)
          ca.apply(g, p, tx0, ty0, wa >> 4, 0, (wa & 15) * 4, L, state,
                   [&](int, uint32_t* h4, uint32_t* m4) { counts(wa, h4, m4); }, &s_wT[wv], &s_wfree[wv],
                   inside ? nullptr : &s_wU[wv]);
        if (eb < nt)
          cb.apply(g, p, tx0, ty0, wb >> 4, 0, (wb & 15) * 4, L, state,
                   [&](int, uint32_t* h4, uint32_t* m4) { counts(wb, h4, m4); }, &s_wT[wv], &s_wfree[wv],
                   inside ? nullptr : &s_wU[wv]);
      }
    } else {
      for (int pass = 0; pass < 4; ++pass) {
        const int ly0 = (lane >> 4) + 16 * pass;
        CellRows<4> sc;
        sc.load_touched(g, tx0, ty0, ly0, 4, hcx, L, state, vec_ok,
                        [&](int ly) { return tq[ly * 16 + (hcx >> 2)] != 0u; });
        sc.apply(g, p, tx0, ty0, ly0, 4, hcx, L, state,
                 [&](int ly, uint32_t* h4, uint32_t* m4) { counts(ly * 16 + (hcx >> 2), h4, m4); },
                 &s_wT[wv], &s_wfree[wv], inside ? nullptr : &s_wU[wv]);
      }
    }
    DM_PH(dm_phase_acc_integrate, 7);
    DM_PH_COUNT(dm_phase_acc_integrate, 21, 1);
    DM_PH_COUNT(dm_phase_acc_integrate, 22, c);
    __builtin_amdgcn_fence(__ATOMIC_ACQ_REL, "wavefront");
    __builtin_amdgcn_wave_barrier();
    if (lane == 0) {
      const int32_t T = s_wT[wv], df = s_wfree[wv];
      const uint32_t U = s_wU[wv] + wU;
      atomicAdd(&s_accT, (unsigned long long)T);
      atomicAdd(&s_accU, (unsigned long long)U);
      if (df) tile_free[tile] = free_update(sfree, df, tile, tlist, tlist_n);
      tile_count[tile] = 0;
      tile_seen[tile] = 1;
      s_wT[wv] = 0;
      s_wfree[wv] = 0;
      s_wU[wv] = 0u;
    }
    for (int e = lane; e < DM_TS * DM_TS / 4; e += 64) tq[e] = 0u;
    __builtin_amdgcn_fence(__ATOMIC_ACQ_REL, "wavefront");
    __builtin_amdgcn_wave_barrier();
  }
  __syncthreads();
  if (tid == 0) {
    unsigned long long* sh = ish + (blockIdx.x % kShards) * kShardWords;
    if (s_accT) atomicAdd(&sh[SH_T], s_accT);
    if (s_accU) atomicAdd(&sh[SH_U], s_accU);
  }
  DM_PH_FLUSH(dm_phase_acc_integrate);
  DM_TL_END(accum, tl_word);
}


__global__ __launch_bounds__(256) void k_integrate_reset(unsigned long long* cnt, unsigned long long* ish) {
  const int i = blockIdx.x * blockDim.x + threadIdx.x;
  constexpr int nI = (int)(sizeof(kIntegrateCounters) / sizeof(kIntegrateCounters[0]));
  if (i < nI) cnt[kIntegrateCounters[i]] = 0ull;
  if (i < kShards * kShardWords) ish[i] = 0ull;
}

constexpr unsigned long long kGateTicks = 500000000ull;

__global__ __launch_bounds__(64) void k_seq_signal(unsigned long long* flag) {
  if (threadIdx.x != 0) return;
  const unsigned long long v = __hip_atomic_load(flag + kSigWord, __ATOMIC_RELAXED, __HIP_MEMORY_SCOPE_AGENT);
  __hip_atomic_store(flag + kSigWord, v + 1, __ATOMIC_RELAXED, __HIP_MEMORY_SCOPE_AGENT);
}

__global__ __launch_bounds__(64) void k_seq_gate(unsigned long long* flag, unsigned long long* err,
                                                 unsigned long long err_bit, unsigned long long ticks,
                                                 unsigned long long fault) {
  if (threadIdx.x != 0) return;
  const unsigned long long seq = flag[kGateWord] + 1;
  flag[kGateWord] = seq;
  const unsigned long long t0 = wall_clock64();
  while (__hip_atomic_load(flag + kSigWord, __ATOMIC_RELAXED, __HIP_MEMORY_SCOPE_AGENT) < seq + fault) {
    __builtin_amdgcn_s_sleep(2);
    if (wall_clock64() - t0 > ticks) {
      atomicOr(err, err_bit);
      return;
    }
  }
}

__device__ inline uint8_t fmask_byte(uint64_t fm, uint64_t um, int j) {
  return (uint8_t)(((fm >> (4 * j)) & 0xFull) | (((um >> (4 * j)) & 0xFull) << 4));
}

__global__ __launch_bounds__(256) void k_recount(Geom g, const int8_t* __restrict__ state,
                                                 int32_t* __restrict__ tile_free, uint8_t* __restrict__ fmask,
                                                 uint64_t* __restrict__ fedge, uint8_t* __restrict__ tile_seen) {
  const int64_t tile = blockIdx.x;
  const int32_t tx0 = (int32_t)(tile % g.r.TX) * DM_TS, ty0 = (int32_t)(tile / g.r.TX) * DM_TS;
  __shared__ int32_t acc, seen;
  __shared__ uint64_t s_edge[4][4];
  if (threadIdx.x == 0) { acc = 0; seen = 0; }
  __syncthreads();
  int32_t c = 0, known = 0;
  uint64_t ew[4] = {0ull, 0ull, 0ull, 0ull};
  uint8_t* tm = fmask + tile * (DM_TS * 16);
  for (int e = threadIdx.x; e < DM_TS * DM_TS; e += 256) {
    const int32_t x = tx0 + (e & 63), y = ty0 + (e >> 6);
    const int8_t b = (x < g.r.W && y < g.r.R) ? state[(int64_t)y * g.r.W + x] : (int8_t)1;
    c += b == 0;
    known |= (x < g.r.W && y < g.r.R && b != -1) ? 1 : 0;
    const uint64_t fm = __ballot(b == 0);
    const uint64_t um = __ballot(b == -1);
    const int l = e & 63, r = e >> 6;
    if (l < 16) tm[r * 16 + l] = fmask_byte(fm, um, l);
    ew[0] |= (um & 1ull) << r;
    ew[1] |= (um >> 63) << r;
    if (r == 0) ew[2] = um;
    if (r == DM_TS - 1) ew[3] = um;
  }
  if (c) atomicAdd(&acc, c);
  if (known) seen = 1;
  const int l4 = __lane_id();
  if (l4 < 4) s_edge[threadIdx.x >> 6][l4] = l4 == 0 ? ew[0] : l4 == 1 ? ew[1] : l4 == 2 ? ew[2] : ew[3];
  __syncthreads();
  if (threadIdx.x == 0) {
    tile_free[tile] = acc;
    tile_seen[tile] = (uint8_t)seen;
  }
  if (threadIdx.x < 4)
    fedge[tile * 4 + threadIdx.x] = s_edge[0][threadIdx.x] | s_edge[1][threadIdx.x] | s_edge[2][threadIdx.x] |
                                    s_edge[3][threadIdx.x];
}

constexpr int kListIters = 16;
__global__ __launch_bounds__(256) void k_list_tiles(int64_t NT, int32_t* __restrict__ tile_free,
                                                    int32_t* __restrict__ ftiles, unsigned long long* list_n,
                                                    int iters) {
  const int lane = __lane_id();
  __shared__ int32_t s_wn[kListIters][4];
  __shared__ unsigned long long s_base;
  const int w = threadIdx.x >> 6;
  const int64_t chunk = (int64_t)iters * blockDim.x;
  for (int64_t c0 = (int64_t)blockIdx.x * chunk; c0 < NT; c0 += (int64_t)gridDim.x * chunk) {
    uint32_t mine = 0u;
    for (int i = 0; i < iters; ++i) {
      const int64_t t = c0 + (int64_t)i * blockDim.x + threadIdx.x;
      if (t >= NT) continue;
      const int32_t v = tile_free[t];
      const bool f = (v & kTileFreeMask) > 0;
      mine |= (f ? 1u : 0u) << i;
      if (f != ((v & kTileListed) != 0)) tile_free[t] = f ? (v | kTileListed) : (v & kTileFreeMask);
    }
    for (int i = 0; i < iters; ++i) {
      const unsigned long long bal = __ballot((mine >> i) & 1u);
      if (lane == 0) s_wn[i][w] = __popcll(bal);
    }
    __syncthreads();
    if (threadIdx.x == 0) {
      int total = 0;
      for (int i = 0; i < iters; ++i) total += s_wn[i][0] + s_wn[i][1] + s_wn[i][2] + s_wn[i][3];
      s_base = total ? atomicAdd(list_n, (unsigned long long)total) : 0ull;
    }
    __syncthreads();
    int64_t pre = (int64_t)s_base;
    for (int i = 0; i < iters; ++i) {
      const bool f = (mine >> i) & 1u;
      const unsigned long long bal = __ballot(f);
      int before = 0;
      for (int q = 0; q < w; ++q) before += s_wn[i][q];
      if (f) {
        const int64_t t = c0 + (int64_t)i * blockDim.x + threadIdx.x;
        ftiles[pre + before + __popcll(bal & ((1ull << lane) - 1ull))] = (int32_t)t;
      }
      pre += s_wn[i][0] + s_wn[i][1] + s_wn[i][2] + s_wn[i][3];
    }
    __syncthreads();
  }
}

__device__ inline uint64_t upto_rows(int p) {
  return p >= 63 ? ~0ull : ((2ull << p) - 1ull);
}

__global__ __launch_bounds__(256) void k_fmask_items(Geom g, const int4* __restrict__ list_a, int cnt_a,
                                                     const int4* __restrict__ list_b, int cnt_b, int cnt_c,
                                                     const PackedPiece* __restrict__ pieces,
                                                     const unsigned long long* __restrict__ cnt,
                                                     const int8_t* __restrict__ state, uint8_t* __restrict__ fmask,
                                                     uint64_t* __restrict__ fedge,
                                                     const unsigned long long* __restrict__ halt) {
  if (*halt) return;
  const int64_t HI = min((int64_t)cnt[cnt_a], g.hitem_cap);
  const int64_t LI = min((int64_t)cnt[cnt_b], (int64_t)g.act_cap);
  const int64_t SI = min((int64_t)cnt[cnt_c], (int64_t)g.act_cap);
  const int lane = __lane_id();
  for (int64_t it = (int64_t)blockIdx.x * 4 + (threadIdx.x >> 6); it < HI + LI + SI;
       it += (int64_t)gridDim.x * 4) {
    const int4 d = it < HI ? list_a[it]
                           : (it < HI + LI ? list_b[it - HI] : list_b[(int64_t)g.act_cap - 1 - (it - HI - LI)]);
    const int32_t tile = __builtin_amdgcn_readfirstlane(d.x);
    uint64_t rows = ~0ull;
    if (it >= HI + LI) {
      const int32_t c0 = __builtin_amdgcn_readfirstlane(d.y);
      const int32_t c = __builtin_amdgcn_readfirstlane(d.z);
      uint64_t mine = 0ull;
      if (lane < c && (int64_t)c0 + c <= g.seg_cap) {
        const PackedPiece q = pieces[c0 + lane];
        const TilePiece tp = dm_unpack_piece(q.x, q.y, q.z, q.w);
        if (tp.len > 0) {
          const int32_t ya = tp.addr0 / kLdsPitch;
          const int32_t yb = dm_piece_addr(tp, tp.len - 1, __builtin_amdgcn_rcpf((float)tp.two_n)) / kLdsPitch;
          const int lo = min(ya, yb), hi = max(ya, yb);
          mine = upto_rows(hi) & ~(lo > 0 ? upto_rows(lo - 1) : 0ull);
        }
      }
      for (int o = 32; o > 0; o >>= 1) mine |= __shfl_xor(mine, o);
      rows = mine;
    }
    const int32_t tx0 = (tile % g.r.TX) * DM_TS, ty0 = (tile / g.r.TX) * DM_TS;
    const int32_t x0 = tx0 + (lane & 3) * 16;
    uint8_t* tm = fmask + (int64_t)tile * (DM_TS * 16);
    EdgeAcc ea;
#pragma unroll
    for (int q = 0; q < 4; ++q) {
      const int ly = 16 * q + (lane >> 2);
      const bool mine = (rows >> ly) & 1ull;
      const int32_t y = ty0 + ly;
      uint32_t out = 0u;
      if (mine && y < g.r.R) {
        const int64_t off = (int64_t)y * g.r.W + x0;
        if (x0 + 16 <= g.r.W && (off & 15) == 0) {
          const uint4 v = *reinterpret_cast<const uint4*>(state + off);
          const uint32_t wd[4] = {v.x, v.y, v.z, v.w};
#pragma unroll
          for (int k = 0; k < 4; ++k) out |= (uint32_t)state_nibbles(wd[k]) << (8 * k);
        } else {
          for (int k = 0; k < 4; ++k) out |= (uint32_t)state_nibbles_at(g, state, x0 + 4 * k, y) << (8 * k);
        }
      }
      if (mine) *reinterpret_cast<uint32_t*>(tm + ly * 16 + (lane & 3) * 4) = out;
      edge_acc(ea, out, q, lane);
    }
    edge_store(ea, fedge, tile, rows, lane);
  }
}

__global__ __launch_bounds__(256) void k_state_from_l(ApplyArgs p, int64_t cells, const float* __restrict__ L,
                                                      int8_t* __restrict__ state) {
  for (int64_t i = (int64_t)blockIdx.x * blockDim.x + threadIdx.x; i < cells;
       i += (int64_t)gridDim.x * blockDim.x)
    state[i] = state_of(p, L[i]);
}

__global__ __launch_bounds__(256) void k_set_state(ApplyArgs p, int64_t cells, const int8_t* __restrict__ in,
                                                   float* __restrict__ L, int8_t* __restrict__ state) {
  for (int64_t i = (int64_t)blockIdx.x * blockDim.x + threadIdx.x; i < cells;
       i += (int64_t)gridDim.x * blockDim.x) {
    const int8_t v = in[i];
    const float l = v == 100 ? p.l_occ : (v == 0 ? p.l_free : 0.0f);
    L[i] = l;
    state[i] = state_of(p, l);
  }
}

__global__ __launch_bounds__(256) void k_map_image(int64_t R, int64_t W, const int8_t* __restrict__ state,
                                                   uint8_t* __restrict__ img) {
  const int64_t cells = R * W;
  for (int64_t i = (int64_t)blockIdx.x * blockDim.x + threadIdx.x; i < cells;
       i += (int64_t)gridDim.x * blockDim.x) {
    const int64_t y = i / W, x = i - y * W;
    const int8_t v = state[i];
    img[(R - 1 - y) * W + x] = v == 0 ? 255 : (v == 100 ? 0 : 127);
  }
}

static_assert(sizeof(Geom) == 72 && sizeof(RayArgs) == 40 && sizeof(ApplyArgs) == 24,
              "kernel argument structs have no implicit padding");

Geom make_geom(const dm_grid* g) {
  Geom ge;
  ge.r.W = (int32_t)g->W;
  ge.r.R = (int32_t)g->R;
  ge.r.row0 = (int32_t)g->row0;
  ge.r.TX = (int32_t)g->TX;
  ge.r.TY = (int32_t)g->TY;
  ge.act_cap = (int32_t)g->act_cap;
  ge.seg_cap = g->segs_cap;
  ge.hitem_cap = g->hitem_cap;
  ge.heavy_cap = g->heavy_cap;
  ge.nb = 0;
  ge.chunks = 1;
  ge.chunk_len = 0;
  ge.sparse_pieces = std::min(g->sparse_pieces, kSparseMax);
  ge.pad = 0;
  return ge;
}

ApplyArgs make_apply(const dm_grid* g) {
  ApplyArgs a;
  a.l_occ = g->p.l_occ;
  a.l_free = g->p.l_free;
  a.l_min = g->p.l_min == 0.0f ? 0.0f : g->p.l_min;
  a.l_max = g->p.l_max == 0.0f ? 0.0f : g->p.l_max;
  a.occ_t = g->p.occ_thresh == 0.0f ? 0.0f : g->p.occ_thresh;
  a.free_t = g->p.free_thresh == 0.0f ? 0.0f : g->p.free_thresh;
  return a;
}

int grid_for(int64_t n, int threads, int64_t cap = 8192) {
  int64_t b = (n + threads - 1) / threads;
  if (b < 1) b = 1;
  if (b > cap) b = cap;
  return (int)b;
}

}

DM_PH_READER(integrate)
DM_TL_READER(accum)

int dm_launch_integrate(dm_grid* g, int32_t S, const double* d_pose4, int32_t N,
                        const float* d_ranges, const double* d_trig) {
  const int64_t nb = (int64_t)S * N;
  g->iw_cur = (g->iw_cur + 1) % dm_grid::kIntSets;
  dm_grid::IntWs& w = g->iw[g->iw_cur];
  hipStream_t fs = g->stream;
  if (g->overlap) {
    fs = g->fe_stream;
    DM_HIP(dm_mark_ws_free(g));
    DM_HIP(hipStreamWaitEvent(fs, w.free_wait ? w.free_wait : w.ev_free, 0));
  }
  DM_LAUNCH(k_integrate_reset, dim3(2), dim3(256), 0, fs, w.cnt, w.sh);
  DM_HIP(hipGetLastError());
  if (nb == 0) {
    if (g->overlap) {
      DM_HIP(hipEventRecord(g->ev_fe, fs));
      DM_HIP(hipStreamWaitEvent(g->stream, g->ev_fe, 0));
      w.free_owed = true;
    }
    return DM_OK;
  }
  RayArgs a;
  a.S = S;
  a.N = N;
  a.ox = g->p.origin_x;
  a.oy = g->p.origin_y;
  a.res = g->p.resolution;
  a.range_min = g->p.range_min;
  a.range_max = g->p.range_max;
  Geom ge = make_geom(g);
  ge.nb = nb;
  ge.chunks = dm_integrate_chunks(g, nb);
  ge.chunk_len = (int32_t)((g->nmax + ge.chunks) / ge.chunks);
  const int nblk = (int)((nb * ge.chunks + 255) / 256);
  KernelTimer t;
  dm_timer_begin(g, "beam_prep", &t, fs);
  DM_LAUNCH(k_beam_prep, dim3(nblk), dim3(256), 0, fs, a, ge, d_pose4, d_ranges,
            d_trig, w.beams, w.tile_count, w.act_raw, w.sh, w.blk_hist, w.blk_n, w.cnt);
  dm_timer_end(g, &t);
  DM_HIP(hipGetLastError());
  dm_timer_begin(g, "plan", &t, fs);
  DM_LAUNCH(k_plan, dim3(grid_for(g->act_cap, kPlanThreads, 256)), dim3(kPlanThreads), 0, fs,
                     ge, w.act_raw, w.sh, w.tile_cur, w.tile_count, w.hitems, w.litems,
                     w.heavy_list, w.cnt);
  dm_timer_end(g, &t);
  DM_HIP(hipGetLastError());
  dm_timer_begin(g, "scatter", &t, fs);
  DM_LAUNCH(k_scatter, dim3(nblk), dim3(256), 0, fs, a, ge, w.beams,
            w.tile_cur, w.blk_hist, w.blk_n, w.pieces, w.cnt);
  dm_timer_end(g, &t);
  DM_HIP(hipGetLastError());
  if (g->overlap) {
    if (int rc = dm_launch_signal(fs, g->fe_flag)) return rc;
    if (int rc = dm_launch_gate(g->stream, g->fe_flag, g->fe_flag + kHaltWord, 1ull,
                                g->fault_gate ? 1000ull : 0ull, g->fault_gate ? (1ull << 40) : 0ull))
      return rc;
  }
  const int vec_ok = (g->W % 4 == 0) ? 1 : 0;
  dm_timer_begin(g, "tile_accum", &t);
  const volatile unsigned long long* hint = g->h_hint;
  const int64_t cap = g->hitem_cap + g->act_cap;
  const int64_t hw = (int64_t)hint[0], hi = (int64_t)hint[1];
  const int64_t accum_wgs = hw > 0 ? std::min(cap, dm_quantize_up(hw + hw / 16 + 64)) : cap;
  DM_LAUNCH(k_tile_accum, dim3(grid_for(accum_wgs, 1, dm_grid::kAccumGrid)),
                     dim3(kQuarter), 0,
                     g->stream, ge, make_apply(g), w.hitems, (int)CNT_ITEMS, w.litems, (int)CNT_LITEMS,
                     (int)CNT_SITEMS, w.pieces, w.tile_count, g->tile_free, w.slabs, g->L, g->state, w.cnt, w.sh, vec_ok,
                     w.heavy_list, w.heavy_done, g->ftiles, g->ftiles_n, g->d_hint, g->fe_flag + kHaltWord,
                     g->tile_seen);
  dm_timer_end(g, &t);
  DM_HIP(hipGetLastError());
  if (g->overlap) w.free_owed = true;
  if (!g->fmask_on) {
    g->fmask_valid = false;
    return DM_OK;
  }
  dm_timer_begin(g, "fmask", &t);
  const int64_t fmask_items = hi > 0 ? std::min(cap, dm_quantize_up(hi + hi / 16 + 64)) : cap;
  DM_LAUNCH(k_fmask_items, dim3(grid_for(fmask_items, 4, 8192)), dim3(256), 0, g->stream,
                     ge, w.hitems, (int)CNT_ITEMS, w.litems, (int)CNT_LITEMS, (int)CNT_SITEMS, w.pieces, w.cnt,
                     g->state, g->fmask, g->fedge,
                     g->fe_flag + kHaltWord);
  dm_timer_end(g, &t);
  DM_HIP(hipGetLastError());
  return DM_OK;
}

int dm_launch_signal(hipStream_t s, unsigned long long* flag) {
  DM_LAUNCH(k_seq_signal, dim3(1), dim3(64), 0, s, flag);
  DM_HIP(hipGetLastError());
  return DM_OK;
}

int dm_launch_gate(hipStream_t s, unsigned long long* flag, unsigned long long* err, unsigned long long err_bit,
                   unsigned long long ticks, unsigned long long fault) {
  DM_LAUNCH(k_seq_gate, dim3(1), dim3(64), 0, s, flag, err, err_bit, ticks ? ticks : kGateTicks, fault);
  DM_HIP(hipGetLastError());
  return DM_OK;
}

int dm_launch_relist(dm_grid* g, bool swap) {
  if (swap) {
    const int x = 1 - g->flist_cur;
    if (g->flist_ev_set[x] && hipEventQuery(g->flist_ev[x]) != hipSuccess)
      DM_HIP(hipStreamWaitEvent(g->stream, g->flist_ev[x], 0));
    if (g->pass_stream) {
      DM_HIP(hipEventRecord(g->flist_ev[g->flist_cur], g->pass_stream));
      g->flist_ev_set[g->flist_cur] = true;
    }
    g->flist_cur = x;
    g->ftiles = g->flist[x];
    g->ftiles_n = g->flist_n[x];
  }
  DM_HIP(hipMemsetAsync(g->ftiles_n, 0, sizeof(unsigned long long), g->stream));
  const int iters = (int)std::min<int64_t>(kListIters, std::max<int64_t>(1, (g->NT + 65535) / 65536));
  DM_LAUNCH(k_list_tiles, dim3(grid_for((g->NT + iters - 1) / iters, 256, 1024)), dim3(256), 0, g->stream,
            g->NT, g->tile_free, g->ftiles, g->ftiles_n, iters);
  DM_HIP(hipGetLastError());
  g->relist_age = 0;
  g->relist_period = swap ? std::min(2 * g->relist_period, kRelistPasses) : 1;
  return DM_OK;
}

int dm_launch_recount(dm_grid* g) {
  const Geom ge = make_geom(g);
  DM_HIP(dm_join_pass_stream(g));
  DM_LAUNCH(k_recount, dim3((unsigned)g->NT), dim3(256), 0, g->stream, ge, g->state,
                     g->tile_free, g->fmask, g->fedge, g->tile_seen);
  DM_HIP(hipGetLastError());
  if (int rc = dm_launch_relist(g, false)) return rc;
  g->fmask_valid = true;
  return DM_OK;
}

int dm_launch_state_from_logodds(dm_grid* g) {
  const int64_t cells = g->R * g->W;
  DM_LAUNCH(k_state_from_l, dim3(grid_for(cells, 256)), dim3(256), 0, g->stream,
                     make_apply(g), cells, g->L, g->state);
  DM_HIP(hipGetLastError());
  return dm_launch_recount(g);
}

int dm_launch_set_state(dm_grid* g, const int8_t* d_in) {
  const int64_t cells = g->R * g->W;
  DM_LAUNCH(k_set_state, dim3(grid_for(cells, 256)), dim3(256), 0, g->stream,
                     make_apply(g), cells, d_in, g->L, g->state);
  DM_HIP(hipGetLastError());
  return dm_launch_recount(g);
}

int dm_launch_map_image(dm_grid* g, uint8_t* d_img) {
  const int64_t cells = g->R * g->W;
  DM_LAUNCH(k_map_image, dim3(grid_for(cells, 256)), dim3(256), 0, g->stream, g->R,
                     g->W, g->state, d_img);
  DM_HIP(hipGetLastError());
  return DM_OK;
}
```

### distributed-autonomous-exploration-and-mapping_amd/csrc/dm_internal.h

```cpp
#pragma once

#include <hip/hip_runtime.h>
#include <stdint.h>

#include <atomic>
#include <chrono>
#include <string>
#include <vector>

#include "../../include/dm.h"

#include "dm_ray.h"


enum {
  CNT_ACTIVE = 0,
  CNT_U = 1,
  CNT_T = 2,
  CNT_SEGS = 3,
  CNT_FTILES = 4,
  CNT_SLOTS = 5,
  CNT_CLUSTERS = 6,
  CNT_OVERFLOW = 7,
  CNT_ITEMS = 8,
  CNT_HEAVY = 9,
  CNT_TH = 10,
  CNT_SORTED = 11,
  CNT_FL0 = 12,
  CNT_STAMP = 13,
  CNT_LITEMS = 14,
  CNT_IOVERFLOW = 15,
  CNT_BIG = 16,
  CNT_SITEMS = 17,
  CNT_N = 18
};
constexpr unsigned long long kOvSlots = 4ull;
constexpr unsigned long long kOvUnionFind = 8ull;
constexpr unsigned long long kOvPipeline = 32ull;
constexpr int kHaltWord = 8;
constexpr int kSigWord = 0;
constexpr int kGateWord = 4;
constexpr int kStampWord = 8;
constexpr int kIntegrateCounters[] = {CNT_ACTIVE, CNT_U, CNT_T, CNT_SEGS, CNT_ITEMS,
                                      CNT_HEAVY, CNT_TH, CNT_LITEMS, CNT_IOVERFLOW, CNT_SITEMS};

constexpr int kIntegrateChunk = 256;
constexpr int kIntegrateMedium = 1024;


constexpr int kShards = 32;
constexpr int kShardWords = 16;
static_assert(kShards * kShardWords == 512, "k_integrate_reset covers 512 shard words");
enum { SH_U = 0, SH_T = 1, SH_TH = 2, SH_ACT = 3 };
enum { SH_SLOT = 0, SH_RUNS = 1, SH_FTF = 2, SH_BIG = 3 };

constexpr int kNStats = 11;
constexpr bool dm_stat_is_frontier(int i) { return i >= 7 && i <= 9; }

constexpr int kRbRecords = 6;
static_assert(kRbRecords * sizeof(dm_cluster) >= (CNT_N + 4) * sizeof(unsigned long long), "readback header");
struct dm_raw_record {
  long long label, size, sum_x, sum_y;
};
constexpr int kRbHostRecords = 6;
static_assert(kRbHostRecords * sizeof(dm_raw_record) >= (CNT_N + 4) * sizeof(unsigned long long),
              "readback header");
__host__ __device__ inline unsigned long long* dm_rb_header(dm_raw_record* records) {
  return reinterpret_cast<unsigned long long*>(records - kRbHostRecords);
}
__host__ __device__ inline const unsigned long long* dm_rb_header(const dm_raw_record* records) {
  return reinterpret_cast<const unsigned long long*>(records - kRbHostRecords);
}
__host__ __device__ inline double dm_centroid(double origin, long long sum, long long size, double res) {
  const double m = (double)sum / (double)size;
  return origin + (m + 0.5) * res;
}

struct dm_grid;
hipError_t dm_copy_shards(dm_grid* g);
inline unsigned long long dm_shard_sum(const unsigned long long* sh, int field) {
  unsigned long long s = 0;
  for (int i = 0; i < kShards; ++i) s += sh[i * kShardWords + field];
  return s;
}

struct KernelTimer {
  std::string name;
  hipEvent_t start, stop;
  hipStream_t stream = nullptr;
};

struct dm_shard_set;

struct dm_grid {
  dm_params p;
  dm_shard_set* sh = nullptr;
  int device = 0;
  int n_cu = 256;
  hipStream_t stream = nullptr;
  bool own_stream = false;
  bool overlap = false;
  hipStream_t fe_stream = nullptr;
  hipEvent_t ev_fe = nullptr;
  unsigned long long* fe_flag = nullptr;
  bool fault_gate = false;
  hipEvent_t ev_bits[2] = {nullptr, nullptr};
  uint64_t integrate_seq = 0;
  struct RbSlot {
    dm_cluster* out_clu = nullptr;
    dm_raw_record* h_out = nullptr;
    dm_raw_record* h_out_dev = nullptr;
    int64_t h_out_cap = 0;
    dm_cluster* m_out = nullptr;
    hipEvent_t ev = nullptr;
    int kind = 0;
    uint64_t seq = 0;
    uint64_t gen = 0;
    uint64_t pass = 0;
    int64_t merge_n = 0;
    uint64_t wepoch = 0, mepoch = 0;
  };
#ifndef DM_RB_SLOTS
#define DM_RB_SLOTS 2
#endif
  static constexpr int kRbSlots = DM_RB_SLOTS;
  static constexpr int kRbSync = kRbSlots;
  RbSlot rb[kRbSlots + 1];
  int rb_head = 0, rb_count = 0;
  int cur_slot = 0;
  uint64_t rb_gen = 0;
  uint64_t fr_pass = 0, m_pass = 0;
  int64_t W = 0, H = 0, R = 0, row0 = 0;
  int64_t TX = 0, TY = 0, NT = 0;
  int32_t nmax = 0;

  float* L = nullptr;
  int8_t* state = nullptr;
  int32_t* tile_free = nullptr;
  uint8_t* fmask = nullptr;
  uint64_t* fedge = nullptr;
  uint8_t* tile_seen = nullptr;
  bool fmask_on = false, fmask_valid = false;
  int fmask_mode = 0;
  unsigned long long* cnt = nullptr;
  unsigned long long* h_cnt = nullptr;
  unsigned long long* fsh = nullptr;
  unsigned long long* h_sh = nullptr;

  int64_t beams_cap = 0;
  int64_t blk_cap = 0;
  int64_t segs_cap = 0;
  int64_t act_cap = 0;
  int64_t hitem_cap = 0;
  int64_t heavy_cap = 0;
  struct IntWs {
    Beam* beams = nullptr;
    int2* blk_hist = nullptr;
    int32_t* blk_n = nullptr;
    int32_t* act_raw = nullptr;
    PackedPiece* pieces = nullptr;
    int4* hitems = nullptr;
    int4* litems = nullptr;
    int32_t* heavy_list = nullptr;
    uint32_t* slabs = nullptr;
    int32_t* heavy_done = nullptr;
    int32_t* tile_count = nullptr;
    int32_t* tile_cur = nullptr;
    unsigned long long* cnt = nullptr;
    unsigned long long* sh = nullptr;
    float* ranges = nullptr;
    int64_t ranges_cap = 0;
    hipEvent_t ev_free = nullptr;
    hipEvent_t free_wait = nullptr;
    bool free_owed = false;
  };
  static constexpr int kIntSets = 2;
  IntWs iw[kIntSets];
  int iw_cur = 0;
  double* trig = nullptr; int32_t trig_n = -1; float trig_amin = 0, trig_inc = 0;
  int64_t trig_cap = 0;
  static constexpr int kPoseRing = 2;
  double* h_pose4[kPoseRing] = {nullptr, nullptr};
  hipEvent_t ev_pose[kPoseRing] = {nullptr, nullptr};
  double* h_pose4_dev[kPoseRing] = {nullptr, nullptr};
  int64_t h_pose_cap = 0;
  int pose_head = 0;
  int32_t last_S = 0, last_N = 0;

  struct FrWs {
    unsigned long long* cnt = nullptr;
    unsigned long long* fsh = nullptr;
    int32_t* big_tiles = nullptr;
    uint64_t* fbits = nullptr;
    int32_t* edge_slot = nullptr;
    int32_t* slot_parent = nullptr;
    hipEvent_t busy = nullptr;
    hipEvent_t ev_split = nullptr;
    bool busy_pending = false;
    uint64_t busy_pass = 0;
  };
  FrWs fw[2];
  unsigned long long* fl_n = nullptr;
  hipStream_t pass_stream = nullptr;
  hipStream_t big_stream = nullptr;
  hipEvent_t ev_bigfork = nullptr, ev_big = nullptr;
  unsigned long long* bits_flag = nullptr;
  hipEvent_t p_tail = nullptr;
  bool p_pending = false;
  uint64_t p_tail_pass = 0;
  int32_t* ftiles = nullptr;
  unsigned long long* ftiles_n = nullptr;
  int32_t* flist[2] = {nullptr, nullptr};
  unsigned long long* flist_n[2] = {nullptr, nullptr};
  hipEvent_t flist_ev[2] = {nullptr, nullptr};
  bool flist_ev_set[2] = {false, false};
  int flist_cur = 0;
  int relist_age = 0;
  int relist_period = 1;
  int32_t* big_tiles = nullptr;
  uint64_t* fbits = nullptr;
  int32_t* border = nullptr;
  unsigned long long* rel = nullptr;
  int32_t fparity = 0;
  int64_t border_cap = 0;
  int64_t slot_cap = 0;
  long long* slot_label = nullptr;
  int32_t* slot_parent = nullptr;
  int32_t* slot_root = nullptr;
  long long* slot_own = nullptr;
  long long* slot_acc = nullptr;
  long long* clusters = nullptr;
  int32_t* slot_k = nullptr;
  int32_t* rank_of = nullptr;
  dm_cluster* out_clu = nullptr;
  dm_raw_record* h_out = nullptr;
  dm_raw_record* h_out_dev = nullptr;
  int64_t h_out_cap = 0;
  int32_t* cell_slot = nullptr;
  int32_t* edge_slot = nullptr;
  long long* edge_label = nullptr;
  uint8_t* mask = nullptr;
  long long* labels = nullptr;
  int8_t* halo = nullptr;
  int has_halo[2] = {0, 0};
  bool frontier_valid = false;

  unsigned long long* bs_key = nullptr;
  unsigned long long* bs_key2 = nullptr;
  int32_t* bs_idx = nullptr;
  int32_t* bs_idx2 = nullptr;
  int64_t bs_cap = 0;
  int32_t* rs_cnt = nullptr;
  int32_t* rs_off = nullptr;
  unsigned long long* rs_status = nullptr;
  int64_t rs_rows = 0;
  int64_t sort_hint = 0, msort_hint = 0;
  int64_t ftile_hint = 0;
  int64_t runs_hint = 0, ftf_hint = 0;
  int64_t big_hint = 0;
  int64_t sort_min = 4096;
  int frontier_kernel = 0;
  static constexpr int kAccumGrid = 16384;
  static constexpr int kChunkThreadsPerCu = 512;
  int sparse_pieces = 15;

  int64_t m_cap = 0;
  int32_t* m_parent = nullptr;
  long long* m_label = nullptr;
  long long* m_acc = nullptr;
  long long* m_clu = nullptr;
  dm_cluster* m_out = nullptr;
  unsigned long long* m_cnt = nullptr;
  unsigned long long* h_mcnt = nullptr;
  unsigned long long* h_hint = nullptr;
  unsigned long long* d_hint = nullptr;

  int goal_slot = -1, goal_kind = 0;
  uint64_t goal_epoch = 0, goal_gen = 0;
  int64_t goal_n = 0;
  unsigned long long* goal_k[2] = {nullptr, nullptr};
  uint32_t* goal_i[2] = {nullptr, nullptr};
  int64_t goal_cap = 0;
  double* goal_io = nullptr;
  int64_t* goal_idx = nullptr;

  uint32_t* plan_cost = nullptr;
  uint64_t* plan_trav = nullptr;
  uint64_t* plan_travs = nullptr;
  int32_t* plan_list[2] = {nullptr, nullptr};
  uint32_t* plan_stamp = nullptr;
  unsigned int* plan_len = nullptr;
  unsigned long long* plan_stat = nullptr;
  unsigned long long* h_plan = nullptr;
  unsigned long long* h_plan_dev = nullptr;
  int64_t* plan_src = nullptr;
  double* plan_qxy = nullptr;
  uint32_t* plan_qcost = nullptr;
  int64_t* plan_qcell = nullptr;
  int64_t plan_qcap = 0;
  int64_t* plan_path = nullptr;
  int64_t plan_pathcap = 0;
  bool plan_valid = false;
  uint64_t plan_version = 0;
  uint64_t reset_seq = 0;
  int64_t plan_max_rounds = 0;

  uint8_t* match_V = nullptr;
  uint8_t* match_kern = nullptr;
  int32_t* match_tiles = nullptr;
  std::vector<uint8_t> match_built;
  std::vector<uint8_t> match_kern_h;
  int32_t match_r = -1;
  uint64_t match_version = 0;
  double* match_pose4 = nullptr;
  int64_t match_pose_cap = 0;
  double* match_trig = nullptr;
  int64_t match_trig_cap = 0;
  float* match_ranges = nullptr;
  int64_t match_ranges_cap = 0;
  int2* match_q = nullptr;
  int64_t match_q_cap = 0;
  uint32_t* match_vol = nullptr;
  int64_t match_vol_cap = 0;
  int32_t* match_out = nullptr;
  int64_t match_out_cap = 0;

  bool profile = false;
  std::vector<KernelTimer> pending;
  std::vector<dm_kernel_stat> stats;
};

inline void dm_select_slot(dm_grid* g, int slot) {
  const dm_grid::RbSlot& r = g->rb[slot];
  g->cur_slot = slot;
  g->out_clu = r.out_clu;
  g->h_out = r.h_out;
  g->h_out_dev = r.h_out_dev;
  g->h_out_cap = r.h_out_cap;
  g->m_out = r.m_out;
}

inline int dm_next_set(const dm_grid* g) { return (g->iw_cur + 1) % dm_grid::kIntSets; }

inline hipError_t dm_mark_ws_free(dm_grid* g, hipEvent_t recorded = nullptr) {
  for (int i = 0; i < dm_grid::kIntSets; ++i) {
    dm_grid::IntWs& w = g->iw[i];
    if (!w.free_owed) continue;
    w.free_owed = false;
    w.free_wait = recorded ? recorded : w.ev_free;
    if (recorded) continue;
    const hipError_t e = hipEventRecord(w.ev_free, g->stream);
    if (e != hipSuccess) return e;
  }
  return hipSuccess;
}

inline void dm_select_fw(dm_grid* g, int s) {
  const dm_grid::FrWs& f = g->fw[s];
  g->cnt = f.cnt;
  g->fsh = f.fsh;
  g->big_tiles = f.big_tiles;
  g->fbits = f.fbits;
  g->edge_slot = f.edge_slot;
  g->slot_parent = f.slot_parent;
}

inline void dm_cpu_relax() {
#if defined(__x86_64__) || defined(__i386__)
  __builtin_ia32_pause();
#elif defined(__aarch64__)
  asm volatile("yield" ::: "memory");
#else
  std::atomic_signal_fence(std::memory_order_seq_cst);
#endif
}

inline hipError_t dm_event_wait(hipEvent_t ev) {
  constexpr long long kSpinNs = 2000000;
  const auto t0 = std::chrono::steady_clock::now();
  for (unsigned it = 0;; ++it) {
    const hipError_t e = hipEventQuery(ev);
    if (e != hipErrorNotReady) return e;
    if ((it & 63u) == 63u &&
        std::chrono::duration_cast<std::chrono::nanoseconds>(std::chrono::steady_clock::now() - t0).count() > kSpinNs)
      return hipEventSynchronize(ev);
    dm_cpu_relax();
  }
}

inline hipError_t dm_join_pass_stream(dm_grid* g) {
  if (!g->p_pending) return hipSuccess;
  g->p_pending = false;
  return hipStreamWaitEvent(g->stream, g->p_tail, 0);
}

inline int32_t dm_integrate_chunks(const dm_grid* g, int64_t nb) {
  const int64_t want = (int64_t)dm_grid::kChunkThreadsPerCu * (int64_t)(g->n_cu > 0 ? g->n_cu : 256);
  if (nb <= 0 || nb >= want) return 1;
  const int64_t by_len = (g->nmax + 1) / 64 > 1 ? (g->nmax + 1) / 64 : 1;
  const int64_t by_fill = (want + nb - 1) / nb;
  return (int32_t)(by_fill < by_len ? by_fill : by_len);
}


int dm_launch_integrate(dm_grid* g, int32_t S, const double* d_pose4, int32_t N,
                        const float* d_ranges, const double* d_trig);
int dm_launch_recount(dm_grid* g);
int dm_launch_relist(dm_grid* g, bool swap);
constexpr int kRelistPasses = 16;
int dm_launch_state_from_logodds(dm_grid* g);
int dm_launch_map_image(dm_grid* g, uint8_t* d_img);
int dm_launch_set_state(dm_grid* g, const int8_t* d_state_in);
int dm_enqueue_frontiers(dm_grid* g, bool want_mask, bool want_labels, bool split = false,
                         hipStream_t* end_stream = nullptr);
int dm_launch_signal(hipStream_t s, unsigned long long* flag);
int dm_launch_gate(hipStream_t s, unsigned long long* flag, unsigned long long* err, unsigned long long err_bit,
                   unsigned long long ticks = 0, unsigned long long fault = 0);
int dm_launch_edge_labels(dm_grid* g);
int dm_frontiers_readback(dm_grid* g, int64_t* n_clusters, int64_t* copied);
int dm_launch_frontiers(dm_grid* g, bool want_mask, bool want_labels, int64_t* n_clusters,
                        int64_t* copied);
int dm_launch_rank_sort(hipStream_t stream, long long* clusters, const long long* sums,
                        const long long* labels, const unsigned long long* d_count,
                        int64_t max_records, double ox, double oy, double res, dm_cluster* out,
                        int32_t* rank_of, unsigned long long* d_sorted, const unsigned long long* cnt,
                        int ncnt, int sorted_idx, const unsigned long long* fsh, dm_raw_record* host_out,
                        int64_t host_cap, int64_t expect);
constexpr int64_t kFmaskOnTiles = 8192;
constexpr int32_t kTileListed = 1 << 30;
constexpr int32_t kTileFreeMask = kTileListed - 1;
constexpr int64_t kSlotsPerTile = 4;
int dm_grow_bucket_sort(dm_grid* g, int64_t n);
int dm_launch_bucket_sort(dm_grid* g, hipStream_t stream, long long* clusters, const long long* sums,
                          const long long* labels, const unsigned long long* d_count,
                          int64_t max_records, int64_t row_base, int64_t rows, dm_cluster* out,
                          int32_t* rank_of, unsigned long long* d_sorted, const unsigned long long* cnt,
                          int ncnt, int sorted_idx, const unsigned long long* fsh, dm_raw_record* host_out,
                          int64_t host_cap);
int64_t dm_export_nbytes(int64_t W, int64_t rec_cap);
int dm_launch_export(dm_grid* g, hipStream_t s, void* d_export, int64_t rec_cap);
int dm_launch_merge(dm_grid* g, hipStream_t s, const void* d_gathered, int32_t nranks, int64_t rec_cap,
                    int64_t min_size);
inline hipStream_t dm_exchange_stream_of(const dm_grid* g) { return g->overlap ? g->pass_stream : g->stream; }
int dm_launch_goal_topk(dm_grid* g, const dm_cluster* d_recs, int64_t K, const double* d_robots, int32_t R,
                        int32_t T, int64_t min_size, double w, double min_dist,
                        const unsigned long long** d_k, const uint32_t** d_i, const uint32_t* d_cost = nullptr);
int dm_plan_launch_travers(dm_grid* g, int32_t inflate_cells);
int dm_plan_launch_expand(dm_grid* g, uint8_t* d_out);
int dm_plan_run_field(dm_grid* g, const int64_t* cells, int32_t n, const int32_t* tiles, int32_t n_tiles,
                      uint32_t max_cost, uint64_t* stats);
int dm_plan_launch_query(dm_grid* g, const double* d_xy, int64_t stride, int64_t n, int32_t snap_cells,
                         uint32_t* d_cost, int64_t* d_cell);
int dm_plan_launch_path(dm_grid* g, const int64_t* d_start, int64_t cap);
int dm_launch_goal_gather(dm_grid* g, const dm_cluster* d_recs, const int64_t* d_idx, int32_t R, double* d_xy);
int dm_match_launch_field(dm_grid* g, int32_t n_tiles, int32_t r, bool mono);
int dm_match_launch_scans(dm_grid* g, int32_t S, int32_t N, int32_t A, int32_t k0, int32_t sub, int32_t half,
                          int32_t stride);
int dm_launch_ld06(dm_grid* g, int32_t S, const dm_ld06_point* d_pts, const int64_t* d_offsets,
                   int32_t N, int dir, float* d_ranges, float* d_intensities);

int dm_sh_destroy(dm_grid* g);
int dm_sh_reset(dm_grid* g);
int dm_sh_integrate(dm_grid* g, int32_t S, const double* poses, int32_t N, const float* ranges, float amin,
                    float inc, uint64_t* U, uint64_t* T);
int dm_sh_integrate_async(dm_grid* g, int32_t S, const double* poses, int32_t N, const float* ranges,
                          float amin, float inc);
int dm_sh_integrate_device(dm_grid* g, int32_t S, const double* d_pose4, int32_t N, const float* d_ranges,
                           float amin, float inc);
int dm_sh_last_counts(dm_grid* g, uint64_t* U, uint64_t* T);
int dm_sh_last_stats(dm_grid* g, uint64_t* out, int32_t cap, int32_t* n_out);
int dm_sh_get_state(dm_grid* g, int8_t* out);
int dm_sh_get_logodds(dm_grid* g, float* out);
int dm_sh_set_logodds(dm_grid* g, const float* in);
int dm_sh_set_state(dm_grid* g, const int8_t* in);
int dm_sh_frontiers(dm_grid* g, uint8_t* mask, int64_t* labels, dm_cluster* out, int64_t cap, int64_t* n_out);
int dm_sh_frontiers_begin(dm_grid* g);
int dm_sh_frontiers_end(dm_grid* g, dm_cluster* out, int64_t cap, int64_t* n_out);
int dm_sh_frontiers_poll(dm_grid* g, int32_t* ready);
int dm_sh_assign_goals(dm_grid* g, const double* robots_xy, int32_t n_robots, int64_t min_size, double w,
                       double min_distance, int64_t* out_index, double* out_xy);
int dm_sh_set_overlap(dm_grid* g, int32_t on);
int dm_sh_synchronize(dm_grid* g);
int dm_sh_profile_enable(dm_grid* g, int enable);
int dm_sh_profile_read(dm_grid* g, dm_kernel_stat* out, int32_t cap, int32_t* n_out);
int dm_sh_profile_reset(dm_grid* g);
int dm_sh_map_image(dm_grid* g, uint8_t* out);
int dm_sh_ld06_to_scans(dm_grid* g, int32_t S, const dm_ld06_point* points, const int64_t* offsets, int32_t N,
                        int dir, float* ranges, float* intensities);
int dm_sh_ld06_to_scans_device(dm_grid* g, int32_t S, const dm_ld06_point* d_points, const int64_t* d_offsets,
                               int32_t N, int dir, float* d_ranges, float* d_intensities);

int dm_set_error(int code, const char* fmt, ...);
int dm_hip_check(hipError_t e, const char* what);
void dm_timer_begin(dm_grid* g, const char* name, KernelTimer* t, hipStream_t s = nullptr);
void dm_timer_end(dm_grid* g, KernelTimer* t);

#define DM_HIP(call)                                         \
  do {                                                       \
    hipError_t _e = (call);                                  \
    if (_e != hipSuccess) return dm_hip_check(_e, #call);    \
  } while (0)

#define DM_LAUNCH(kernel, grid, block, shmem, stream, ...) \
  hipLaunchKernelGGL(kernel, grid, block, shmem, stream, __VA_ARGS__)

inline int64_t dm_quantize_up(int64_t n) {
  if (n <= 8) return n;
  int sh = 0;
  while ((n >> sh) >= 8) ++sh;
  const int64_t step = (int64_t)1 << sh;
  return ((n + step - 1) / step) * step;
}
```

Before: 209.4 billion.

## Write ray pieces directly in beam_prep via per-tile run tables, drop scatter pass

Beam preparation now writes packed pieces straight into a per-block region of the pieces buffer. Each tile records up to 32 runs (address delta and offset) in a run table, and overflow runs go to a separate list that a small gather kernel compacts. This removes the separate scatter kernel, the stored Beam array and the per-block histograms, so beams are no longer recomputed and re-walked in a second pass. The cost is that work items become larger records carrying run tables, and consumers must do a binary-search run lookup on every piece access. Piece storage is also over-allocated per block, and the tile counter widens to 64 bits.

```diff
diff --git a/distributed-autonomous-exploration-and-mapping_amd/csrc/dm_api.cpp b/distributed-autonomous-exploration-and-mapping_amd/csrc/dm_api.cpp
--- a/distributed-autonomous-exploration-and-mapping_amd/csrc/dm_api.cpp
+++ b/distributed-autonomous-exploration-and-mapping_amd/csrc/dm_api.cpp
@@ -112,26 +112,23 @@
   const int64_t chunks = dm_integrate_chunks(g, nb);
   const int64_t per_beam = 2 * (g->nmax / DM_TILE) + 8 + 4 * chunks;
   const int64_t blocks = ceil_div(nb * chunks, 256);
-  if (nb > g->beams_cap || blocks > g->blk_cap) {
-    const int64_t nbc = std::max<int64_t>(nb, g->beams_cap);
-    const int64_t bc = std::max<int64_t>(blocks, g->blk_cap);
+  if (blocks > g->blk_cap) {
     int rc = 0;
+    for (auto& w : g->iw)
+      if (!rc) rc = dev_alloc(&w.ov_runs, blocks * 1024, "overflow run list");
+    if (rc) { g->blk_cap = 0; return rc; }
+    g->blk_cap = blocks;
+  }
+  const int64_t segs = nb * per_beam;
+  const int64_t seg_alloc = blocks * dm_block_pieces(g, (int32_t)chunks) + segs;
+  if (seg_alloc > (int64_t)0x7FFFFFFF)
+    return dm_set_error(DM_ERR_CAPACITY, "batch too large: %lld pieces", (long long)seg_alloc);
+  if (seg_alloc > g->segs_cap) {
     for (auto& w : g->iw) {
-      if (!rc) rc = dev_alloc(&w.beams, nbc, "beams");
-      if (!rc) rc = dev_alloc(&w.blk_hist, bc * 1024, "per-block tile histograms");
-      if (!rc) rc = dev_alloc(&w.blk_n, bc, "per-block histogram sizes");
-    }
-    if (rc) { g->beams_cap = g->blk_cap = 0; return rc; }
-    g->beams_cap = nbc;
-    g->blk_cap = bc;
-  }
-  const int64_t segs = nb * per_beam;
-  if (segs > g->segs_cap) {
-    for (auto& w : g->iw) {
-      int rc = dev_alloc(&w.pieces, segs, "ray pieces");
+      int rc = dev_alloc(&w.pieces, seg_alloc, "ray pieces");
       if (rc) { g->segs_cap = 0; return rc; }
     }
-    g->segs_cap = segs;
+    g->segs_cap = seg_alloc;
   }
   const int64_t side = ceil_div(2 * (int64_t)g->nmax + 1, DM_TILE) + 1;
   int64_t act = std::min<int64_t>(g->NT, std::min<int64_t>(segs, (int64_t)S * side * side));
@@ -369,7 +366,7 @@
   if (rc) return rc;
   const unsigned long long* ic = g->h_cnt + CNT_N;
   if (ic[CNT_IOVERFLOW]) {
-    (void)hipMemset(g->iw[g->iw_cur].tile_count, 0, sizeof(int32_t) * (size_t)g->NT);
+    (void)hipMemset(g->iw[g->iw_cur].tile_count, 0, sizeof(unsigned long long) * (size_t)g->NT);
     return dm_set_error(DM_ERR_CAPACITY, "integrate workspace overflow (flags %llu: 1 first-touch "
                         "list, 2 pieces, 4 work lists)",
                         (unsigned long long)ic[CNT_IOVERFLOW]);
@@ -477,7 +474,10 @@
   if ((rc = dev_alloc(&g->state, cells, "state"))) return fail(rc);
   for (auto& w : g->iw) {
     if ((rc = dev_alloc(&w.tile_count, g->NT, "tile counts"))) return fail(rc);
-    if ((rc = dev_alloc(&w.tile_cur, g->NT, "tile bin cursors"))) return fail(rc);
+    if ((rc = dev_alloc(&w.run_tab, g->NT * kTileRuns, "tile run tables"))) return fail(rc);
+    if ((rc = dev_alloc(&w.run_len, g->NT * kTileRuns, "tile run lengths"))) return fail(rc);
+    if ((rc = dev_alloc(&w.tile_bin, g->NT, "gathered tile bins"))) return fail(rc);
+    if ((rc = dev_alloc(&w.fe_cur, kFeWords, "front-end cursors"))) return fail(rc);
     if ((rc = dev_alloc(&w.cnt, CNT_N, "integrate counters"))) return fail(rc);
     if ((rc = dev_alloc(&w.sh, kShards * kShardWords, "integrate shard counters"))) return fail(rc);
     DM_HIP(hipMemset(w.cnt, 0, sizeof(unsigned long long) * CNT_N));
@@ -611,9 +611,9 @@
   dev_free(g->match_out);
   for (auto& w : g->iw) {
     dev_free(w.pieces); dev_free(w.hitems); dev_free(w.litems); dev_free(w.heavy_list); dev_free(w.slabs);
-    dev_free(w.heavy_done); dev_free(w.tile_count); dev_free(w.tile_cur); dev_free(w.cnt); dev_free(w.sh);
+    dev_free(w.heavy_done); dev_free(w.tile_count); dev_free(w.run_tab); dev_free(w.run_len); dev_free(w.tile_bin); dev_free(w.fe_cur); dev_free(w.cnt); dev_free(w.sh);
     dev_free(w.ranges);
-    dev_free(w.beams); dev_free(w.blk_hist); dev_free(w.blk_n); dev_free(w.act_raw);
+    dev_free(w.ov_runs); dev_free(w.act_raw);
   }
   dev_free(g->L); dev_free(g->state); dev_free(g->fmask); dev_free(g->fedge); dev_free(g->tile_seen);
   dev_free(g->tile_free);
@@ -647,7 +647,7 @@
   DM_HIP(hipMemsetAsync(g->L, 0, sizeof(float) * (size_t)cells, g->stream));
   DM_HIP(hipMemsetAsync(g->state, 0xFF, (size_t)cells, g->stream));
   DM_HIP(dm_sync_all(g));
-  for (auto& w : g->iw) DM_HIP(hipMemsetAsync(w.tile_count, 0, sizeof(int32_t) * (size_t)g->NT, g->stream));
+  for (auto& w : g->iw) DM_HIP(hipMemsetAsync(w.tile_count, 0, sizeof(unsigned long long) * (size_t)g->NT, g->stream));
   DM_HIP(hipMemsetAsync(g->tile_free, 0, sizeof(int32_t) * (size_t)g->NT, g->stream));
   if ((rc = dm_launch_recount(g))) return rc;
   for (auto& f : g->fw) DM_HIP(hipMemsetAsync(f.cnt, 0, sizeof(unsigned long long) * CNT_N, g->stream));
diff --git a/distributed-autonomous-exploration-and-mapping_amd/csrc/dm_integrate.hip b/distributed-autonomous-exploration-and-mapping_amd/csrc/dm_integrate.hip
--- a/distributed-autonomous-exploration-and-mapping_amd/csrc/dm_integrate.hip
+++ b/distributed-autonomous-exploration-and-mapping_amd/csrc/dm_integrate.hip
@@ -18,7 +18,7 @@
   int64_t nb;
   int32_t chunks, chunk_len;
   int32_t sparse_pieces;
-  int32_t pad;
+  int32_t ov_cap;
 };
 
 struct BeamChunk {
@@ -106,52 +106,123 @@
   return dm_pack_piece(dm_tile_piece(bm, k0, k1, g.r.row0, tx0, ty0, kLdsPitch));
 }
 
-__global__ __launch_bounds__(256) void k_beam_prep(RayArgs a, Geom g, const double* __restrict__ pose4,
+__device__ inline void publish_run(const Geom& g, int32_t tile, unsigned long long old, int32_t addr, int32_t len,
+                                   ItemRun* __restrict__ run_tab, int32_t* __restrict__ run_len,
+                                   TileRun* __restrict__ ov_runs, unsigned long long* fe_cur, int32_t* act_raw,
+                                   unsigned long long* ish, unsigned long long* cnt) {
+  const int32_t off = dm_word_pieces(old), ord = dm_word_runs(old);
+  first_touch(g, tile, ord, act_raw, ish, cnt);
+  if (ord < kTileRuns) {
+    ItemRun r;
+    r.delta = addr - off; r.off = off;
+    run_tab[(int64_t)tile * kTileRuns + ord] = r;
+    run_len[(int64_t)tile * kTileRuns + ord] = len;
+  } else {
+    TileRun r;
+    r.addr = addr; r.off = off; r.len = len; r.aux = tile;
+    const unsigned long long n = atomicAdd(&fe_cur[FE_OVN], 1ull);
+    if (n < (unsigned long long)g.ov_cap) ov_runs[n] = r;
+    else atomicOr(&cnt[CNT_IOVERFLOW], 4ull);
+  }
+}
+
+__global__ __launch_bounds__(256) void k_beam_prep(RayArgs a, Geom g, int32_t blk_range,
+                                                   const double* __restrict__ pose4,
                                                    const float* __restrict__ ranges,
                                                    const double* __restrict__ trig,
-                                                   Beam* __restrict__ beams, int32_t* tile_count,
-                                                   int32_t* act_raw, unsigned long long* ish,
-                                                   int2* __restrict__ blk_hist, int32_t* __restrict__ blk_n,
+                                                   unsigned long long* tile_count, int32_t* act_raw,
+                                                   unsigned long long* ish, ItemRun* __restrict__ run_tab,
+                                                   int32_t* __restrict__ run_len, TileRun* __restrict__ ov_runs,
+                                                   unsigned long long* fe_cur, PackedPiece* __restrict__ pieces,
                                                    unsigned long long* cnt) {
   __shared__ int32_t hkey[kHash];
   __shared__ int32_t hcnt[kHash];
-  __shared__ int32_t s_nh;
-  const int tid = threadIdx.x;
+  __shared__ int32_t hoff[kHash];
+  __shared__ int32_t s_wsum[4];
+  __shared__ int32_t s_xn, s_xcur;
+  const int tid = threadIdx.x, lane = lane_id();
+  DM_PH_INIT();
   for (int e = tid; e < kHash; e += 256) { hkey[e] = -1; hcnt[e] = 0; }
-  if (tid == 0) s_nh = 0;
+  if (tid == 0) s_xn = 0;
   __syncthreads();
   const int64_t v = (int64_t)blockIdx.x * blockDim.x + tid;
-  if (v < g.nb * g.chunks) {
-    const BeamChunk bc = beam_chunk(g, v);
-    const int32_t s = (int32_t)(bc.b / a.N), i = (int32_t)(bc.b % a.N);
-    const Beam bm = dm_make_beam(a, pose4, ranges, trig, s, i);
-    if (bc.k_lo == 0) beams[bc.b] = bm;
-    if ((bm.flags & 1) && bc.k_lo <= bm.n) {
-      dm_for_each_piece(bm, g.r, [&](int32_t tile, int32_t, int32_t) {
-        const LaneRun run = lane_run(tile);
-        if (run.head) {
-          const int h = hash_insert(hkey, tile);
-          if (h >= 0) {
-            atomicAdd(&hcnt[h], run.len);
-          } else {
-            const int32_t old = atomicAdd(&tile_count[tile], run.len);
-            first_touch(g, tile, old, act_raw, ish, cnt);
-          }
-        }
-      }, bc.k_lo, bc.k_hi);
-    }
+  const bool in = v < g.nb * g.chunks;
+  const BeamChunk bc = beam_chunk(g, in ? v : 0);
+  Beam bm;
+  bm.flags = 0;
+  if (in) bm = dm_make_beam(a, pose4, ranges, trig, (int32_t)(bc.b / a.N), (int32_t)(bc.b % a.N));
+  const bool valid = in && (bm.flags & 1) && bc.k_lo <= bm.n;
+  DM_PH(dm_phase_acc_integrate, 8);
+  if (valid) {
+    dm_for_each_piece(bm, g.r, [&](int32_t tile, int32_t, int32_t) {
+      const LaneRun run = lane_run(tile);
+      if (run.head) {
+        const int h = hash_insert(hkey, tile);
+        atomicAdd(h >= 0 ? &hcnt[h] : &s_xn, run.len);
+      }
+    }, bc.k_lo, bc.k_hi);
   }
   __syncthreads();
-  int2* my_hist = blk_hist + (int64_t)blockIdx.x * kHash;
-  for (int e = tid; e < kHash; e += 256) {
-    const int32_t tile = hkey[e];
-    if (tile < 0) continue;
-    const int32_t old = atomicAdd(&tile_count[tile], hcnt[e]);
-    first_touch(g, tile, old, act_raw, ish, cnt);
-    my_hist[atomicAdd(&s_nh, 1)] = make_int2(tile, hcnt[e] | (e << 16));
-  }
+  DM_PH(dm_phase_acc_integrate, 9);
+  int32_t c4[4], sum = 0;
+#pragma unroll
+  for (int j = 0; j < 4; ++j) { c4[j] = hcnt[4 * tid + j]; sum += c4[j]; }
+  int32_t incl = sum;
+  for (int d = 1; d < 64; d <<= 1) {
+    const int32_t t = __shfl_up(incl, d);
+    if (lane >= d) incl += t;
+  }
+  if (lane == 63) s_wsum[tid >> 6] = incl;
   __syncthreads();
-  if (tid == 0) blk_n[blockIdx.x] = s_nh;
+  const int32_t hashed = s_wsum[0] + s_wsum[1] + s_wsum[2] + s_wsum[3];
+  if (hashed + s_xn > blk_range || (int64_t)(blockIdx.x + 1) * blk_range > g.seg_cap) {
+    if (tid == 0) atomicOr(&cnt[CNT_IOVERFLOW], 2ull);
+    return;
+  }
+  if (hashed + s_xn == 0) return;
+  const int32_t base = (int32_t)blockIdx.x * blk_range;
+  int32_t ft[4];
+  unsigned long long old[4];
+#pragma unroll
+  for (int j = 0; j < 4; ++j) {
+    const int e = tid + 256 * j;
+    ft[j] = hkey[e];
+    old[j] = 0ull;
+    if (ft[j] >= 0) old[j] = atomicAdd(&tile_count[ft[j]], dm_run_word(hcnt[e]));
+  }
+  int32_t pre = incl - sum;
+  for (int w = 0; w < (tid >> 6); ++w) pre += s_wsum[w];
+#pragma unroll
+  for (int j = 0; j < 4; ++j) { hoff[4 * tid + j] = pre; pre += c4[j]; }
+  if (tid == 0) s_xcur = hashed;
+  __syncthreads();
+  DM_PH(dm_phase_acc_integrate, 10);
+  if (valid) {
+    dm_for_each_piece(bm, g.r, [&](int32_t tile, int32_t k0, int32_t k1) {
+      const LaneRun run = lane_run(tile);
+      int32_t pos = 0;
+      if (run.head) {
+        const int h = hash_find(hkey, tile);
+        pos = base + atomicAdd(h >= 0 ? &hoff[h] : &s_xcur, run.len);
+        if (h < 0)
+          publish_run(g, tile, atomicAdd(&tile_count[tile], dm_run_word(run.len)), pos, run.len, run_tab, run_len,
+                      ov_runs, fe_cur, act_raw, ish, cnt);
+      }
+      pos = __shfl(pos, run.head_lane);
+      pieces[pos + run.rank] = make_piece(g, bm, tile, k0, k1);
+    }, bc.k_lo, bc.k_hi);
+  }
+  __syncthreads();
+  DM_PH(dm_phase_acc_integrate, 11);
+#pragma unroll
+  for (int j = 0; j < 4; ++j) {
+    const int e = tid + 256 * j;
+    if (ft[j] >= 0)
+      publish_run(g, ft[j], old[j], base + hoff[e] - hcnt[e], hcnt[e], run_tab, run_len, ov_runs, fe_cur, act_raw,
+                  ish, cnt);
+  }
+  DM_PH(dm_phase_acc_integrate, 12);
+  DM_PH_FLUSH(dm_phase_acc_integrate);
 }
 
 constexpr int kChunk = kIntegrateChunk;
@@ -195,11 +266,14 @@
   }
 }
 
-__global__ __launch_bounds__(kPlanThreads) void k_plan(Geom g, const int32_t* __restrict__ act_raw,
+__global__ __launch_bounds__(kPlanThreads) void k_plan(Geom g, int64_t bin0, const int32_t* __restrict__ act_raw,
                                                        const unsigned long long* __restrict__ ish,
-                                                       int32_t* __restrict__ tile_cur,
-                                                       const int32_t* __restrict__ tile_count,
-                                                       int4* __restrict__ hitems, int4* __restrict__ litems,
+                                                       const unsigned long long* __restrict__ tile_count,
+                                                       const ItemRun* __restrict__ run_tab,
+                                                       const int32_t* __restrict__ run_len,
+                                                       int32_t* __restrict__ tile_bin, TileRun* __restrict__ ov_runs,
+                                                       unsigned long long* fe_cur,
+                                                       ItemRec* __restrict__ hitems, ItemRec* __restrict__ litems,
                                                        int32_t* __restrict__ heavy_list,
                                                        unsigned long long* cnt) {
   __shared__ int32_t soff[kShards + 1];
@@ -220,7 +294,11 @@
   const int64_t stride = (int64_t)gridDim.x * blockDim.x;
   for (int64_t j0 = (int64_t)blockIdx.x * blockDim.x + (tid & ~63); j0 < n; j0 += stride) {
     const int64_t j = j0 + lane;
-    int32_t t = -1, c = 0;
+    int32_t t = -1, c = 0, nr = 0;
+    int4 rw[kTileRuns / 2];
+    constexpr int kEager = 4;
+#pragma unroll
+    for (int k = 0; k < kTileRuns / 2; ++k) rw[k] = make_int4(0, kNoRun, 0, kNoRun);
     if (j < n) {
       int a = 0, b = kShards - 1;
       while (a < b) {
@@ -228,8 +306,48 @@
         if (soff[mid] <= j) a = mid; else b = mid - 1;
       }
       t = act_raw[(int64_t)a * g.act_cap + (j - soff[a])];
-      c = tile_count[t];
-    }
+      const unsigned long long w = tile_count[t];
+      const int4* tr = reinterpret_cast<const int4*>(run_tab + (int64_t)t * kTileRuns);
+#pragma unroll
+      for (int k = 0; k < kEager; ++k) rw[k] = tr[k];
+      c = dm_word_pieces(w);
+      nr = dm_word_runs(w);
+      if (nr > 2 * kEager && nr <= kTileRuns) {
+#pragma unroll
+        for (int k = kEager; k < kTileRuns / 2; ++k)
+          if (2 * k < nr) rw[k] = tr[k];
+      }
+    }
+    if (nr > kTileRuns) {
+      const unsigned long long b0 = (unsigned long long)bin0 + atomicAdd(&fe_cur[FE_CUR], (unsigned long long)c);
+      int32_t bin = -1;
+      if ((int64_t)(b0 + (unsigned long long)c) <= g.seg_cap) {
+        bin = (int32_t)b0;
+        const unsigned long long l0 = atomicAdd(&fe_cur[FE_OVN], (unsigned long long)kTileRuns);
+        if ((int64_t)l0 + kTileRuns <= (int64_t)g.ov_cap) {
+          for (int k = 0; k < kTileRuns; ++k) {
+            const ItemRun r = run_tab[(int64_t)t * kTileRuns + k];
+            TileRun o;
+            o.addr = r.delta + r.off; o.off = r.off; o.len = run_len[(int64_t)t * kTileRuns + k]; o.aux = t;
+            ov_runs[l0 + k] = o;
+          }
+        } else {
+          atomicOr(&cnt[CNT_IOVERFLOW], 4ull);
+        }
+      } else {
+        atomicOr(&cnt[CNT_IOVERFLOW], 2ull);
+      }
+      tile_bin[t] = bin;
+      rw[0].x = max(bin, 0);
+      rw[0].y = 0;
+      nr = 1;
+    }
+#pragma unroll
+    for (int k = 0; k < kTileRuns / 2; ++k) {
+      if (2 * k >= nr) { rw[k].x = 0; rw[k].y = kNoRun; }
+      if (2 * k + 1 >= nr) { rw[k].z = 0; rw[k].w = kNoRun; }
+    }
+    const uint32_t wmask = dm_run_write_mask(nr);
     const bool heavy = c > kMedium;
     const bool medium = c > kChunk && !heavy;
     const bool sparse = t >= 0 && c <= g.sparse_pieces;
@@ -241,78 +359,60 @@
                                         sparse ? 1ull : 0ull, heavy ? 1ull : 0ull};
     unsigned long long got[5];
     wave_alloc_n<5>(ctr, want, got);
-    const unsigned long long p0 = got[0], hi = got[1], li = got[2], si = got[3], ho = got[4];
+    const unsigned long long hi = got[1], li = got[2], si = got[3], ho = got[4];
     if (t < 0) continue;
-    tile_cur[t] = (int32_t)p0;
-    const bool fits = (int64_t)(p0 + c) <= g.seg_cap && (int64_t)(hi + nh_items) <= g.hitem_cap &&
+    const bool fits = (int64_t)(hi + nh_items) <= g.hitem_cap &&
                       (int64_t)li < (int64_t)g.act_cap && (int64_t)si < (int64_t)g.act_cap &&
                       (int64_t)ho < g.heavy_cap;
     if (!fits) {
       atomicOr(&cnt[CNT_IOVERFLOW], 4ull);
       continue;
     }
+    auto put_item = [&](ItemRec* dst, int32_t first, int32_t pieces, int32_t code) {
+      int4* d4 = reinterpret_cast<int4*>(dst);
+      d4[0] = make_int4(t, first, pieces, code);
+#pragma unroll
+      for (int k = 0; k < kTileRuns / 2; ++k)
+        if ((wmask >> k) & 1u) d4[1 + k] = rw[k];
+    };
     if (sparse) {
-      litems[(int64_t)g.act_cap - 1 - (int64_t)si] = make_int4(t, (int32_t)p0, c, -1);
+      put_item(litems + ((int64_t)g.act_cap - 1 - (int64_t)si), 0, c, -1);
     } else if (light) {
-      litems[li] = make_int4(t, (int32_t)p0, c, -1);
+      put_item(litems + li, 0, c, -1);
     } else if (medium) {
-      hitems[hi] = make_int4(t, (int32_t)p0, c, -1);
+      put_item(hitems + hi, 0, c, -1);
     } else {
       const int32_t wide = c >= 65536 ? 1 : 0;
       heavy_list[ho] = t | (wide << 31);
       for (int32_t q = 0; q < nh_items; ++q)
-        hitems[hi + q] = make_int4(t, (int32_t)p0 + q * kChunk, min(kChunk, c - q * kChunk),
-                                   (int32_t)(2 * ho + wide));
-    }
-  }
-}
-
-__device__ inline void put_piece(const Geom& g, PackedPiece* pieces, int64_t idx, const Beam& bm,
-                                 int32_t tile, int32_t k0, int32_t k1, unsigned long long* cnt) {
-  if (idx >= 0 && idx < g.seg_cap) {
-    pieces[idx] = make_piece(g, bm, tile, k0, k1);
-  } else {
-    atomicOr(&cnt[CNT_IOVERFLOW], 2ull);
-  }
-}
-
-__global__ __launch_bounds__(256) void k_scatter(RayArgs a, Geom g, const Beam* __restrict__ beams,
-                                                 int32_t* tile_cur, const int2* __restrict__ blk_hist,
-                                                 const int32_t* __restrict__ blk_n,
-                                                 PackedPiece* __restrict__ pieces, unsigned long long* cnt) {
-  __shared__ int32_t hkey[kHash];
-  __shared__ int32_t hcnt[kHash];
-  __shared__ int32_t hbase[kHash];
-  const int tid = threadIdx.x;
-  for (int e = tid; e < kHash; e += 256) { hkey[e] = -1; hcnt[e] = 0; }
-  const int64_t v = (int64_t)blockIdx.x * blockDim.x + tid;
-  const bool in = v < g.nb * g.chunks;
-  const BeamChunk bc = beam_chunk(g, in ? v : 0);
-  Beam bm;
-  bm.flags = 0;
-  if (in) bm = beams[bc.b];
-  const int32_t nh = blk_n[blockIdx.x];
-  __syncthreads();
-  const int2* my_hist = blk_hist + (int64_t)blockIdx.x * kHash;
-  for (int e = tid; e < nh; e += 256) {
-    const int2 te = my_hist[e];
-    const int h = hash_insert(hkey, te.x);
-    if (h >= 0) hbase[h] = atomicAdd(&tile_cur[te.x], te.y & 0xFFFF);
-  }
-  __syncthreads();
-  const bool valid = in && (bm.flags & 1) && bc.k_lo <= bm.n;
-  if (valid) {
-    dm_for_each_piece(bm, g.r, [&](int32_t tile, int32_t k0, int32_t k1) {
-      const LaneRun run = lane_run(tile);
-      int32_t pos = -1;
-      if (run.head) {
-        const int h = hash_find(hkey, tile);
-        pos = h >= 0 ? hbase[h] + atomicAdd(&hcnt[h], run.len) : atomicAdd(&tile_cur[tile], run.len);
-      }
-      pos = __shfl(pos, run.head_lane);
-      put_piece(g, pieces, (int64_t)pos + run.rank, bm, tile, k0, k1, cnt);
-    }, bc.k_lo, bc.k_hi);
-  }
+        put_item(hitems + (hi + q), q * kChunk, min(kChunk, c - q * kChunk), (int32_t)(2 * ho + wide));
+    }
+  }
+}
+
+__global__ __launch_bounds__(kPlanThreads) void k_gather_signal(Geom g, const int32_t* __restrict__ tile_bin,
+                                                               const TileRun* __restrict__ ov_runs,
+                                                               const unsigned long long* __restrict__ fe_cur,
+                                                               PackedPiece* pieces, unsigned long long* sig) {
+  const int64_t n = min((int64_t)fe_cur[FE_OVN], (int64_t)g.ov_cap);
+  const int lane = __lane_id();
+  for (int64_t e = threadIdx.x >> 6; e < n; e += kPlanThreads / 64) {
+    const TileRun r = ov_runs[e];
+    if (r.aux < 0 || r.aux >= g.r.TX * g.r.TY) continue;
+    const int64_t bin = tile_bin[r.aux];
+    const int64_t dst = bin + r.off;
+    if (bin < 0 || r.off < 0 || r.addr < 0 || r.len < 0 || (int64_t)r.addr + r.len > g.seg_cap || dst + r.len > g.seg_cap)
+      continue;
+    for (int32_t i = lane; i < r.len; i += 64) pieces[dst + i] = pieces[r.addr + i];
+  }
+  if (!sig) return;
+  if (n > 0) {
+    __threadfence();
+    __syncthreads();
+  }
+  if (threadIdx.x != 0) return;
+  const unsigned long long v = __hip_atomic_load(sig + kSigWord, __ATOMIC_RELAXED, __HIP_MEMORY_SCOPE_AGENT);
+  __hip_atomic_store(sig + kSigWord, v + 1, __ATOMIC_RELAXED, __HIP_MEMORY_SCOPE_AGENT);
 }
 
 struct ApplyArgs {
@@ -592,6 +692,17 @@
   return sp.n;
 }
 
+__device__ inline int4 item_desc(const ItemRec* __restrict__ rec) { return *reinterpret_cast<const int4*>(rec); }
+__device__ inline ItemRun load_runs(const ItemRec* __restrict__ rec, int lane) {
+  uint32_t off = 16u + 8u * ((uint32_t)lane & (uint32_t)(kTileRuns - 1));
+  asm volatile("" : "+v"(off));
+  return *reinterpret_cast<const ItemRun*>(reinterpret_cast<const char*>(rec) + off);
+}
+__device__ inline int32_t run_piece(const ItemRun& run, int32_t i, int64_t seg_cap) {
+  return dm_run_lookup([&](int k) { return __shfl(run.off, k); }, [&](int k) { return __shfl(run.delta, k); }, i,
+                       seg_cap);
+}
+
 __device__ inline PackedPiece no_piece() {
   PackedPiece q;
   q.x = 0u; q.y = 0u; q.z = 0u; q.w = 1u;
@@ -609,7 +720,7 @@
 }
 
 __device__ inline void finish_tile(const Geom& g, int32_t tile, int32_t T, int32_t dfree, uint32_t U,
-                                   bool heavy, int32_t* tile_count, int32_t* tile_free, int32_t old_free,
+                                   bool heavy, unsigned long long* tile_count, int32_t* tile_free, int32_t old_free,
                                    int32_t* tlist, unsigned long long* tlist_n, unsigned long long* ish) {
   unsigned long long* sh = ish + (blockIdx.x % kShards) * kShardWords;
   if (T) {
@@ -618,7 +729,7 @@
   }
   if (U) atomicAdd(&sh[SH_U], (unsigned long long)U);
   if (dfree) tile_free[tile] = free_update(old_free, dfree, tile, tlist, tlist_n);
-  tile_count[tile] = 0;
+  tile_count[tile] = 0ull;
 }
 
 __device__ inline void heavy_quarter(const Geom& g, const ApplyArgs& p, int64_t h, int q, int32_t tile,
@@ -680,8 +791,8 @@
 #endif
 constexpr int kAccumPerCu = DM_ACCUM_OCC;
 __global__ __launch_bounds__(kQuarter, kAccumPerCu) void k_tile_accum(
-    Geom g, ApplyArgs p, const int4* __restrict__ list_a, int cnt_a, const int4* __restrict__ list_b,
-    int cnt_b, int cnt_c, const PackedPiece* __restrict__ pieces, int32_t* tile_count, int32_t* tile_free,
+    Geom g, ApplyArgs p, const ItemRec* __restrict__ list_a, int cnt_a, const ItemRec* __restrict__ list_b,
+    int cnt_b, int cnt_c, const PackedPiece* __restrict__ pieces, unsigned long long* tile_count, int32_t* tile_free,
     uint32_t* __restrict__ slabs, float* __restrict__ L, int8_t* __restrict__ state,
     const unsigned long long* __restrict__ cnt, unsigned long long* ish, int vec_ok,
     const int32_t* __restrict__ heavy_list, int32_t* heavy_done, int32_t* tlist, unsigned long long* tlist_n,
@@ -713,9 +824,13 @@
     return;
   }
   auto item_of = [&](int64_t it) {
-    int4 d = it < n_items ? (it < HI ? list_a[it] : list_b[it - HI]) : make_int4(0, 0, 0, -1);
-    d.z = (int64_t)d.y + d.z <= g.seg_cap ? d.z : 0;
-    return d;
+    return it < n_items ? item_desc(it < HI ? list_a + it : list_b + (it - HI)) : make_int4(0, 0, 0, -1);
+  };
+  auto runs_of = [&](int64_t it) {
+    ItemRun r;
+    r.delta = 0; r.off = kNoRun;
+    if (it < n_items) r = load_runs(it < HI ? list_a + it : list_b + (it - HI), lane);
+    return r;
   };
   const int cx = (tid & 15) * 4;
   __shared__ unsigned long long s_accT, s_accU;
@@ -732,12 +847,12 @@
   auto piece_of = [&](int32_t f) -> int32_t {
     return f == 1 ? tid : dm_udiv_small(tid, f, __builtin_amdgcn_rcpf((float)f));
   };
-  auto load_pieces = [&](const int4& d) -> PackedPiece {
+  auto load_pieces = [&](const int4& d, const ItemRun& r) -> PackedPiece {
     const int32_t c0 = __builtin_amdgcn_readfirstlane(d.y);
     const int32_t c = __builtin_amdgcn_readfirstlane(d.z);
-    return pieces[c0 + min(piece_of(split_of(d)), max(c - 1, 0))];
+    return pieces[run_piece(r, c0 + min(piece_of(split_of(d)), max(c - 1, 0)), g.seg_cap)];
   };
-  mine = load_pieces(info);
+  mine = load_pieces(info, runs_of(blockIdx.x));
   PackedPiece mine_n = mine;
   for (int e = tid; e < kTileWords; e += kQuarter) tl[e] = 0u;
   if (tid == 0) { s_T = 0; s_free = 0; s_U = 0u; s_accT = 0ull; s_accU = 0ull; }
@@ -754,7 +869,7 @@
     DM_PH(dm_phase_acc_integrate, 0);
     if (heavy >= 0) {
       walk_piece(tl, mine, tid < c, lane);
-      mine_n = load_pieces(next);
+      mine_n = load_pieces(next, runs_of(it + G));
       __syncthreads();
       DM_PH(dm_phase_acc_integrate, 1);
       DM_PH_COUNT(dm_phase_acc_integrate, 17, 1);
@@ -777,7 +892,7 @@
       asm volatile("s_waitcnt vmcnt(0)" ::: "memory");
       __syncthreads();
       if (tid == 0) {
-        const int32_t n_it = (tile_count[tile] + kChunk - 1) / kChunk;
+        const int32_t n_it = (dm_word_pieces(tile_count[tile]) + kChunk - 1) / kChunk;
         s_last = atomicAdd(&heavy_done[heavy >> 1], 1) == n_it - 1;
       }
       __syncthreads();
@@ -812,7 +927,8 @@
       } else {
         u = walk_piece(tl, mine, tid < c, lane);
         for (int32_t r0 = kChunk; r0 < c; r0 += kChunk) {
-          const PackedPiece more = r0 + tid < c ? pieces[c0 + r0 + tid] : no_piece();
+          const int32_t at = run_piece(runs_of(it), c0 + min(r0 + tid, c - 1), g.seg_cap);
+          const PackedPiece more = r0 + tid < c ? pieces[at] : no_piece();
           u += walk_piece(tl, more, r0 + tid < c, lane);
         }
       }
@@ -821,7 +937,7 @@
         for (int o = 32; o > 0; o >>= 1) u += __shfl_xor(u, o);
         if (lane == 0) atomicAdd(&s_U, (uint32_t)u);
       }
-      mine_n = load_pieces(next);
+      mine_n = load_pieces(next, runs_of(it + G));
       __syncthreads();
       DM_PH(dm_phase_acc_integrate, 3);
       DM_PH_COUNT(dm_phase_acc_integrate, 16, 1);
@@ -842,7 +958,7 @@
       s_accT += (unsigned long long)s_T;
       s_accU += (unsigned long long)s_U;
       if (s_free) tile_free[tile] = free_update(tfree, s_free, tile, tlist, tlist_n);
-      tile_count[tile] = 0;
+      tile_count[tile] = 0ull;
       tile_seen[tile] = 1;
     }
     info = next;
@@ -855,21 +971,23 @@
   __shared__ int32_t s_wT[kQuarter / 64], s_wfree[kQuarter / 64];
   __shared__ uint32_t s_wU[kQuarter / 64];
   __shared__ uint16_t s_list[kQuarter / 64][kSparseList];
-  const int wv = tid >> 6;
+  const int wv = __builtin_amdgcn_readfirstlane(tid >> 6);
   uint32_t* tq = tl + wv * (DM_TS * DM_TS / 4);
   const int hcx = (lane & 15) * 4;
   if (lane == 0) { s_wT[wv] = 0; s_wfree[wv] = 0; s_wU[wv] = 0u; }
   const int nw = kQuarter / 64;
   for (int64_t it = sp_rank * nw + wv; it < SI; it += (int64_t)G * nw) {
-    int4 d = list_b[(int64_t)g.act_cap - 1 - it];
-    d.z = (int64_t)d.y + d.z <= g.seg_cap ? d.z : 0;
+    const ItemRec* srec = list_b + ((int64_t)g.act_cap - 1 - it);
+    const int4 d = item_desc(srec);
+    const ItemRun srun = load_runs(srec, lane);
     const int32_t tile = d.x, c0 = d.y, c = d.z;
     if (lane == 0 && wv == 0) tl_word += 1ull << 16;
     const int32_t tx0 = (tile % g.r.TX) * DM_TS, ty0 = (tile / g.r.TX) * DM_TS;
     const int32_t fs = dm_split_factor(c, 64);
     const float rfs = __builtin_amdgcn_rcpf((float)fs);
     const int32_t spi = fs == 1 ? lane : dm_udiv_small(lane, fs, rfs);
-    const PackedPiece sp = spi < c ? pieces[c0 + spi] : no_piece();
+    const int32_t sat = run_piece(srun, c0 + min(spi, max(c - 1, 0)), g.seg_cap);
+    const PackedPiece sp = spi < c ? pieces[sat] : no_piece();
     const int32_t sfree = tile_free[tile];
     int32_t u = walk_piece_bytes(tq, sp, spi < c, fs, lane - spi * fs, rfs);
     const bool inside = tx0 + DM_TS <= g.r.W && ty0 + DM_TS <= g.r.R;
@@ -943,7 +1061,7 @@
       atomicAdd(&s_accT, (unsigned long long)T);
       atomicAdd(&s_accU, (unsigned long long)U);
       if (df) tile_free[tile] = free_update(sfree, df, tile, tlist, tlist_n);
-      tile_count[tile] = 0;
+      tile_count[tile] = 0ull;
       tile_seen[tile] = 1;
       s_wT[wv] = 0;
       s_wfree[wv] = 0;
@@ -964,11 +1082,13 @@
 }
 
 
-__global__ __launch_bounds__(256) void k_integrate_reset(unsigned long long* cnt, unsigned long long* ish) {
+__global__ __launch_bounds__(256) void k_integrate_reset(unsigned long long* cnt, unsigned long long* ish,
+                                                         unsigned long long* fe_cur) {
   const int i = blockIdx.x * blockDim.x + threadIdx.x;
   constexpr int nI = (int)(sizeof(kIntegrateCounters) / sizeof(kIntegrateCounters[0]));
   if (i < nI) cnt[kIntegrateCounters[i]] = 0ull;
   if (i < kShards * kShardWords) ish[i] = 0ull;
+  if (i < kFeWords) fe_cur[i] = 0ull;
 }
 
 constexpr unsigned long long kGateTicks = 500000000ull;
@@ -1089,8 +1209,8 @@
   return p >= 63 ? ~0ull : ((2ull << p) - 1ull);
 }
 
-__global__ __launch_bounds__(256) void k_fmask_items(Geom g, const int4* __restrict__ list_a, int cnt_a,
-                                                     const int4* __restrict__ list_b, int cnt_b, int cnt_c,
+__global__ __launch_bounds__(256) void k_fmask_items(Geom g, const ItemRec* __restrict__ list_a, int cnt_a,
+                                                     const ItemRec* __restrict__ list_b, int cnt_b, int cnt_c,
                                                      const PackedPiece* __restrict__ pieces,
                                                      const unsigned long long* __restrict__ cnt,
                                                      const int8_t* __restrict__ state, uint8_t* __restrict__ fmask,
@@ -1103,16 +1223,19 @@
   const int lane = __lane_id();
   for (int64_t it = (int64_t)blockIdx.x * 4 + (threadIdx.x >> 6); it < HI + LI + SI;
        it += (int64_t)gridDim.x * 4) {
-    const int4 d = it < HI ? list_a[it]
-                           : (it < HI + LI ? list_b[it - HI] : list_b[(int64_t)g.act_cap - 1 - (it - HI - LI)]);
+    const ItemRec* rec =
+        it < HI ? list_a + it : (it < HI + LI ? list_b + (it - HI) : list_b + ((int64_t)g.act_cap - 1 - (it - HI - LI)));
+    const int4 d = item_desc(rec);
     const int32_t tile = __builtin_amdgcn_readfirstlane(d.x);
     uint64_t rows = ~0ull;
     if (it >= HI + LI) {
       const int32_t c0 = __builtin_amdgcn_readfirstlane(d.y);
       const int32_t c = __builtin_amdgcn_readfirstlane(d.z);
+      const ItemRun srun = load_runs(rec, lane);
+      const int32_t at = run_piece(srun, c0 + min(lane, max(c - 1, 0)), g.seg_cap);
       uint64_t mine = 0ull;
-      if (lane < c && (int64_t)c0 + c <= g.seg_cap) {
-        const PackedPiece q = pieces[c0 + lane];
+      if (lane < c) {
+        const PackedPiece q = pieces[at];
         const TilePiece tp = dm_unpack_piece(q.x, q.y, q.z, q.w);
         if (tp.len > 0) {
           const int32_t ya = tp.addr0 / kLdsPitch;
@@ -1199,7 +1322,7 @@
   ge.chunks = 1;
   ge.chunk_len = 0;
   ge.sparse_pieces = std::min(g->sparse_pieces, kSparseMax);
-  ge.pad = 0;
+  ge.ov_cap = (int32_t)std::min<int64_t>(g->blk_cap * 1024, 0x7FFFFFFF);
   return ge;
 }
 
@@ -1237,7 +1360,7 @@
     DM_HIP(dm_mark_ws_free(g));
     DM_HIP(hipStreamWaitEvent(fs, w.free_wait ? w.free_wait : w.ev_free, 0));
   }
-  DM_LAUNCH(k_integrate_reset, dim3(2), dim3(256), 0, fs, w.cnt, w.sh);
+  DM_LAUNCH(k_integrate_reset, dim3(2), dim3(256), 0, fs, w.cnt, w.sh, w.fe_cur);
   DM_HIP(hipGetLastError());
   if (nb == 0) {
     if (g->overlap) {
@@ -1260,25 +1383,25 @@
   ge.chunks = dm_integrate_chunks(g, nb);
   ge.chunk_len = (int32_t)((g->nmax + ge.chunks) / ge.chunks);
   const int nblk = (int)((nb * ge.chunks + 255) / 256);
+  const int32_t blk_range = dm_block_pieces(g, ge.chunks);
   KernelTimer t;
   dm_timer_begin(g, "beam_prep", &t, fs);
-  DM_LAUNCH(k_beam_prep, dim3(nblk), dim3(256), 0, fs, a, ge, d_pose4, d_ranges,
-            d_trig, w.beams, w.tile_count, w.act_raw, w.sh, w.blk_hist, w.blk_n, w.cnt);
+  DM_LAUNCH(k_beam_prep, dim3(nblk), dim3(256), 0, fs, a, ge, blk_range, d_pose4, d_ranges,
+            d_trig, w.tile_count, w.act_raw, w.sh, w.run_tab, w.run_len, w.ov_runs, w.fe_cur, w.pieces, w.cnt);
   dm_timer_end(g, &t);
   DM_HIP(hipGetLastError());
   dm_timer_begin(g, "plan", &t, fs);
   DM_LAUNCH(k_plan, dim3(grid_for(g->act_cap, kPlanThreads, 256)), dim3(kPlanThreads), 0, fs,
-                     ge, w.act_raw, w.sh, w.tile_cur, w.tile_count, w.hitems, w.litems,
-                     w.heavy_list, w.cnt);
+                     ge, (int64_t)nblk * blk_range, w.act_raw, w.sh, w.tile_count, w.run_tab, w.run_len, w.tile_bin,
+                     w.ov_runs, w.fe_cur, w.hitems, w.litems, w.heavy_list, w.cnt);
   dm_timer_end(g, &t);
   DM_HIP(hipGetLastError());
-  dm_timer_begin(g, "scatter", &t, fs);
-  DM_LAUNCH(k_scatter, dim3(nblk), dim3(256), 0, fs, a, ge, w.beams,
-            w.tile_cur, w.blk_hist, w.blk_n, w.pieces, w.cnt);
+  dm_timer_begin(g, "gather_signal", &t, fs);
+  DM_LAUNCH(k_gather_signal, dim3(1), dim3(kPlanThreads), 0, fs, ge, w.tile_bin, w.ov_runs, w.fe_cur, w.pieces,
+            g->overlap ? g->fe_flag : nullptr);
   dm_timer_end(g, &t);
   DM_HIP(hipGetLastError());
   if (g->overlap) {
-    if (int rc = dm_launch_signal(fs, g->fe_flag)) return rc;
     if (int rc = dm_launch_gate(g->stream, g->fe_flag, g->fe_flag + kHaltWord, 1ull,
                                 g->fault_gate ? 1000ull : 0ull, g->fault_gate ? (1ull << 40) : 0ull))
       return rc;
diff --git a/distributed-autonomous-exploration-and-mapping_amd/csrc/dm_internal.h b/distributed-autonomous-exploration-and-mapping_amd/csrc/dm_internal.h
--- a/distributed-autonomous-exploration-and-mapping_amd/csrc/dm_internal.h
+++ b/distributed-autonomous-exploration-and-mapping_amd/csrc/dm_internal.h
@@ -11,6 +11,7 @@
 #include "../../include/dm.h"
 
 #include "dm_ray.h"
+#include "dm_runs.h"
 
 
 enum {
@@ -51,6 +52,7 @@
 constexpr int kShards = 32;
 constexpr int kShardWords = 16;
 static_assert(kShards * kShardWords == 512, "k_integrate_reset covers 512 shard words");
+enum { FE_CUR = 0, FE_OVN = 1, kFeWords = 2 };
 enum { SH_U = 0, SH_T = 1, SH_TH = 2, SH_ACT = 3 };
 enum { SH_SLOT = 0, SH_RUNS = 1, SH_FTF = 2, SH_BIG = 3 };
 
@@ -147,25 +149,25 @@
   unsigned long long* fsh = nullptr;
   unsigned long long* h_sh = nullptr;
 
-  int64_t beams_cap = 0;
   int64_t blk_cap = 0;
   int64_t segs_cap = 0;
   int64_t act_cap = 0;
   int64_t hitem_cap = 0;
   int64_t heavy_cap = 0;
   struct IntWs {
-    Beam* beams = nullptr;
-    int2* blk_hist = nullptr;
-    int32_t* blk_n = nullptr;
     int32_t* act_raw = nullptr;
+    ItemRun* run_tab = nullptr;
+    int32_t* run_len = nullptr;
+    int32_t* tile_bin = nullptr;
+    TileRun* ov_runs = nullptr;
+    unsigned long long* fe_cur = nullptr;
     PackedPiece* pieces = nullptr;
-    int4* hitems = nullptr;
-    int4* litems = nullptr;
+    ItemRec* hitems = nullptr;
+    ItemRec* litems = nullptr;
     int32_t* heavy_list = nullptr;
     uint32_t* slabs = nullptr;
     int32_t* heavy_done = nullptr;
-    int32_t* tile_count = nullptr;
-    int32_t* tile_cur = nullptr;
+    unsigned long long* tile_count = nullptr;
     unsigned long long* cnt = nullptr;
     unsigned long long* sh = nullptr;
     float* ranges = nullptr;
@@ -403,6 +405,11 @@
 }
 
 
+inline int32_t dm_block_pieces(const dm_grid* g, int32_t chunks) {
+  const int64_t len = chunks > 1 ? (g->nmax + chunks) / chunks : g->nmax;
+  return (int32_t)(256 * (2 * (len / DM_TILE) + 8 + 4));
+}
+
 int dm_launch_integrate(dm_grid* g, int32_t S, const double* d_pose4, int32_t N,
                         const float* d_ranges, const double* d_trig);
 int dm_launch_recount(dm_grid* g);
diff --git a/distributed-autonomous-exploration-and-mapping_amd/csrc/dm_runs.h b/distributed-autonomous-exploration-and-mapping_amd/csrc/dm_runs.h
--- /dev/null
+++ b/distributed-autonomous-exploration-and-mapping_amd/csrc/dm_runs.h
@@ -0,0 +1,51 @@
+#pragma once
+
+#include <stdint.h>
+
+#include "dm_ray.h"
+
+constexpr int kTileRuns = 32;
+constexpr int32_t kNoRun = 0x7FFFFFFF;
+
+struct TileRun {
+  int32_t addr;
+  int32_t off;
+  int32_t len;
+  int32_t aux;
+};
+static_assert(sizeof(TileRun) == 16, "TileRun layout");
+
+struct ItemRun {
+  int32_t delta;
+  int32_t off;
+};
+static_assert(sizeof(ItemRun) == 8, "ItemRun layout");
+
+struct ItemRec {
+  int32_t tile, first, pieces, code;
+  ItemRun run[kTileRuns];
+};
+static_assert(sizeof(ItemRec) == 16 + 8 * kTileRuns, "ItemRec layout");
+
+DM_HD inline unsigned long long dm_run_word(int32_t pieces) { return (unsigned long long)(uint32_t)pieces | (1ull << 32); }
+DM_HD inline int32_t dm_word_pieces(unsigned long long w) { return (int32_t)(uint32_t)w; }
+DM_HD inline int32_t dm_word_runs(unsigned long long w) { return (int32_t)(uint32_t)(w >> 32); }
+
+static_assert((kTileRuns & (kTileRuns - 1)) == 0, "dm_run_lookup bisects");
+template <class OffAt, class DeltaAt>
+DM_HD inline int32_t dm_run_lookup(OffAt&& off_at, DeltaAt&& delta_at, int32_t i, int64_t seg_cap) {
+  int k = 0;
+  for (int step = kTileRuns / 2; step > 0; step >>= 1)
+    if (i >= off_at(k + step)) k += step;
+  const uint32_t idx = (uint32_t)(i + delta_at(k)), last = (uint32_t)(seg_cap - 1);
+  return (int32_t)(idx < last ? idx : last);
+}
+
+DM_HD inline uint32_t dm_run_write_mask(int32_t nr) {
+  uint32_t words = nr >= kTileRuns ? 0xFFFFFFFFu : (1u << ((nr + 1) / 2)) - 1u;
+  for (int step = kTileRuns / 2; step > 0; step >>= 1) {
+    const int32_t p = ((nr - 1) & ~(2 * step - 1)) + step;
+    if (p >= nr) words |= 1u << (p / 2);
+  }
+  return words & (uint32_t)((1ull << (kTileRuns / 2)) - 1ull);
+}
```

Result: slower. 200.2 billion (-4.4%).
